# max-andr/joint-cnn-mrf

Measured on AMD Instinct MI355X. Metric: images/sec (720x480, K=9 joints) part-detector+spatial-model fwd, higher is better.
Workload: dtype f32(fp16x2 spectra, fft); 1 GPU; configs[1]: batch=64/GPU synthetic 480x720x3, part detector + spatial model forward + argmax, fp32; batch_per_gpu=64, global_batch=64, micro_batch=64, use_sm=True, collective=all_gather coords int32 [B,2,9]

## Files before the change

### joint-cnn-mrf_amd/csrc/conv_fft.hip

```cpp
#include <cmath>
#include <map>
#include <mutex>
#include <utility>
#include <vector>

#include "conv_fft_common.h"
#include "conv_fft_plan.h"

namespace jcm {
namespace cfft {

template <int KS, int NP>
__global__ __launch_bounds__(256) void weight_spectra_split_kernel(const float* __restrict__ w, uint4* __restrict__ Ws, int Cin, int Cout, int CoutP, int ntl, int NY, int NX,
                                                                   int round_bf16, float* __restrict__ wscale) {
  __shared__ cf twy[192][KS - 1], twx[KS];
  const int tid = threadIdx.x;
  const int kx = blockIdx.y;
#pragma unroll 1
  for (int k = tid; k < NY * (KS - 1) + KS; k += 256) {
    const bool isy = k < NY * (KS - 1);
    const int ky = k / (KS - 1), a = isy ? k % (KS - 1) + 1 : k - NY * (KS - 1);
    const int num = isy ? (ky * a) % NY : (kx * a) % NX, den = isy ? NY : NX;
    double sn, cs;
    sincospi(-2.0 * (double)num / (double)den, &sn, &cs);
    cf* dstw = isy ? &twy[ky][a - 1] : &twx[a];
    *dstw = cf{(float)cs, (float)sn};
  }
  __syncthreads();
  constexpr int CPT = 8;
  constexpr int NPP = NP == 5 ? 1 : 2;
  static_assert(NP == 2 || NP == 4 || NP == 5, "operand forms of the channel GEMM");
  float wmul = 1.f;
  if constexpr (NP >= 4) {
    int ex = 0;
    const float bound = wscale[0];
    if (bound > 0.f && bound < 3.0e38f) (void)frexpf(bound, &ex);
    wmul = ldexpf(1.f, 14 - ex);
    if (blockIdx.x == 0 && blockIdx.y == 0 && threadIdx.x == 0) wscale[1] = ldexpf(1.f, ex - 14);
  }
  const size_t e = (size_t)blockIdx.x * 256 + tid;
  if (e >= (size_t)(Cin / CPT) * CoutP) return;
  const int co = (int)(e % CoutP), cig = (int)(e / CoutP);
  cf ra[CPT][KS];
  const unsigned toff = (unsigned)(cig * CPT * Cout + (co < Cout ? co : Cout - 1));
#pragma unroll
  for (int c = 0; c < CPT; ++c)
#pragma unroll
    for (int a = 0; a < KS; ++a) ra[c][a] = cf{0.f, 0.f};
#pragma unroll 1
  for (int a = 0; a < KS; ++a) {
    cf sum[CPT];
#pragma unroll
    for (int c = 0; c < CPT; ++c) sum[c] = cf{0.f, 0.f};
#pragma unroll
    for (int b = 0; b < KS; ++b) {
      const float* tap = w + (size_t)((KS - 1 - a) * KS + (KS - 1 - b)) * Cin * Cout;
      const cf tw = twx[b];
#pragma unroll
      for (int c = 0; c < CPT; ++c) {
        float wv = tap[toff + (unsigned)(c * Cout)];
        wv = co < Cout ? wv : 0.f;
        if (round_bf16) wv = static_cast<float>(static_cast<__bf16>(wv));
        sum[c] = sfma(wv, tw, sum[c]);
      }
    }
#pragma unroll
    for (int c = 0; c < CPT; ++c)
#pragma unroll
      for (int aa = 0; aa < KS; ++aa) ra[c][aa] = aa == a ? sum[c] : ra[c][aa];
  }
  const int KC = Cin / 16, ntiles = CoutP / ntl;
  const int ci0 = cig * CPT, kc = ci0 >> 4, kg = (ci0 >> 3) & 1, nt = co / ntl, sn = co % ntl;
  const size_t fstride = NP == 5 ? (size_t)ntiles * (KC >> 1) * 8 * ntl : (size_t)ntiles * KC * (4 * NPP) * ntl;
  uint4* dst = Ws + (size_t)kx * NY * fstride +
               (NP == 5 ? ((size_t)nt * (KC >> 1) + (kc >> 1)) * 8 * ntl + ((size_t)(kc & 1) * 2 + kg) * ntl + sn :
                          ((size_t)nt * KC + kc) * (4 * NPP) * ntl + (size_t)kg * ntl + sn);
  typedef unsigned u32x4n __attribute__((ext_vector_type(4)));
  auto put = [](uint4* q, const uint4& v) __attribute__((always_inline)) { __builtin_nontemporal_store(u32x4n{v.x, v.y, v.z, v.w}, reinterpret_cast<u32x4n*>(q)); };
  auto emit = [&](uint4* d, const float (&xr)[CPT], const float (&xi)[CPT]) __attribute__((always_inline)) {
    if constexpr (NP == 5) {
      float x8[8];
#pragma unroll
      for (int c = 0; c < 8; ++c) x8[c] = xr[c % CPT];
      put(d, round8h(x8, wmul));
#pragma unroll
      for (int c = 0; c < 8; ++c) x8[c] = xi[c % CPT];
      put(d + (size_t)4 * ntl, round8h(x8, wmul));
    } else {
      uint4 u[NPP];
      float x8[8];
#pragma unroll
      for (int c = 0; c < 8; ++c) x8[c] = xr[c % CPT];
      if constexpr (NP == 4) split8h(x8, wmul, u);
      else split8<NPP>(x8, u);
#pragma unroll
      for (int p = 0; p < NPP; ++p) put(d + (size_t)p * 2 * ntl, u[p]);
#pragma unroll
      for (int c = 0; c < 8; ++c) x8[c] = xi[c % CPT];
      if constexpr (NP == 4) split8h(x8, wmul, u);
      else split8<NPP>(x8, u);
#pragma unroll
      for (int p = 0; p < NPP; ++p) put(d + (size_t)(NPP + p) * 2 * ntl, u[p]);
    }
  };
  for (int ky = 0; ky <= NY / 2; ++ky) {
    const int kp = ky == 0 ? 0 : NY - ky;
    float cs[KS - 1], sn_[KS - 1];
#pragma unroll
    for (int a = 1; a < KS; ++a) { const cf t = twy[ky][a - 1]; cs[a - 1] = t.x; sn_[a - 1] = -t.y; }
    float xr[CPT], xi[CPT], pr[CPT], pi_[CPT];
#pragma unroll
    for (int c = 0; c < CPT; ++c) {
      cf C = ra[c][0], S = cf{0.f, 0.f};
#pragma unroll
      for (int a = 1; a < KS; ++a) { C = sfma(cs[a - 1], ra[c][a], C); S = sfma(sn_[a - 1], ra[c][a], S); }
      xr[c] = C.x + S.y; xi[c] = C.y - S.x;
      pr[c] = C.x - S.y; pi_[c] = C.y + S.x;
    }
    emit(dst + (size_t)ky * fstride, xr, xi);
    if (kp != ky) emit(dst + (size_t)kp * fstride, pr, pi_);
  }
}

template <int TAPS>
__global__ __launch_bounds__(256) void weight_bound_kernel(const float* __restrict__ w, size_t pairs, int round_bf16, float* __restrict__ wmax) {
  __shared__ float red[4];
  float m = 0.f;
  for (size_t e = (size_t)blockIdx.x * 256 + threadIdx.x; e < pairs; e += (size_t)gridDim.x * 256) {
    float v[TAPS];
#pragma unroll
    for (int t = 0; t < TAPS; ++t) v[t] = w[(size_t)t * pairs + e];
    float sum = 0.f;
#pragma unroll
    for (int t = 0; t < TAPS; ++t) {
      float x = v[t];
      if (round_bf16) x = static_cast<float>(static_cast<__bf16>(x));
      sum += fabsf(x);
    }
    m = fmaxf(m, sum);
  }
  block_max_to<256>(m * 1.0001f, wmax, red, threadIdx.x);
}

struct Sizes { int NY, NX; };
static const int kLens[] = {20, 24, 28, 32, 36, 40, 50, 60, 64, 72, 96, 100, 128, 192};
static bool pick(int need, int* n) {
  for (int v : kLens)
    if (v >= need) { *n = v; return true; }
  return false;
}
static int tw_offset(int n) {
  int off = 0;
  for (int v : kLens) {
    if (v == n) return off;
    off += v;
  }
  return -1;
}
static bool sizes_of(int H, int W, int ks, Sizes* s, int circ = 0) {
  if (circ) {
    s->NY = H; s->NX = W;
    return (ks == 9 || ks == 5) && H > 8 && W > 8 && tw_offset(H) >= 0 && tw_offset(W) >= 0;
  }
  return (ks == 9 || ks == 5) && H + ks - 1 <= 192 && W + ks - 1 <= 192 && pick(H + 4, &s->NY) && pick(W + 4, &s->NX);
}
static int pad64(int c) { return (c + CB - 1) / CB * CB; }
static int padn(int c, int n) { return (c + n - 1) / n * n; }

int persistent_grid(const void* kernel, int ntiles, int threads, int dyn_lds) {
  static std::mutex mu;
  static std::map<std::pair<const void*, int>, int> cache;
  int dev = 0;
  (void)hipGetDevice(&dev);
  int resident = 0;
  {
    std::lock_guard<std::mutex> lk(mu);
    auto it = cache.find({kernel, dev});
    if (it != cache.end()) resident = it->second;
  }
  if (!resident) {
    int ncu = 256, per_cu = 0;
    (void)hipDeviceGetAttribute(&ncu, hipDeviceAttributeMultiprocessorCount, dev);
    if (hipOccupancyMaxActiveBlocksPerMultiprocessor(&per_cu, kernel, threads, (size_t)dyn_lds) != hipSuccess || per_cu < 1) per_cu = 1;
    resident = ncu * per_cu;
    std::lock_guard<std::mutex> lk(mu);
    cache[{kernel, dev}] = resident;
  }
  return resident < ntiles ? resident : ntiles;
}

static const cf* twiddle_table(int dev) {
  static std::mutex mu;
  static std::map<int, cf*> tabs;
  std::lock_guard<std::mutex> lk(mu);
  auto it = tabs.find(dev);
  if (it != tabs.end()) return it->second;
  std::vector<float> h;
  for (int n : kLens)
    for (int k = 0; k < n; ++k) {
      const double ang = 2.0 * 3.14159265358979323846 * (double)k / (double)n;
      h.push_back((float)std::cos(ang));
      h.push_back((float)std::sin(ang));
    }
  cf* d = nullptr;
  if (hipMalloc(reinterpret_cast<void**>(&d), h.size() * sizeof(float)) != hipSuccess) return nullptr;
  if (hipMemcpy(d, h.data(), h.size() * sizeof(float), hipMemcpyHostToDevice) != hipSuccess) { (void)hipFree(d); return nullptr; }
  tabs[dev] = d;
  return d;
}

}

using namespace cfft;

bool conv_fft_supported(const ConvArgs& a, int ks, int circ) {
  Sizes s;
  return a.Cin % CB == 0 && a.Cin >= CB && a.Cout >= 1 && a.B >= 1 && sizes_of(a.H, a.W, ks, &s, circ);
}
static bool operand_form(int np) { return np == kFftBf16x2 || np == kFftFp16x2 || np == kFftFp16x1; }
size_t conv_fft_weight_bytes(int H, int W, int ks, int Cin, int Cout, int np, int circ) {
  Sizes s;
  if (!sizes_of(H, W, ks, &s, circ)) return 0;
  return cgemm_split_w_bytes(np, s.NY * (s.NX / 2 + 1), Cin, Cout);
}
hipError_t conv_fft_pack_weights(const float* w_hwio, void* wf, int H, int W, int ks, int Cin, int Cout, int np, bool round_bf16, hipStream_t st, float* wscale, int circ,
                                 const float* bound_from) {
  Sizes s;
  if (!sizes_of(H, W, ks, &s, circ) || Cin % 16 || !operand_form(np) || (np >= 4 && !wscale) || (np == kFftFp16x1 && Cin % 32)) return hipErrorInvalidValue;
  const int ntl = cgemm_split_ntile(np, Cout), CoutP = padn(Cout, ntl);
  const size_t cpt = 8;
  const dim3 grid((unsigned)(((size_t)Cin / cpt * CoutP + 255) / 256), (unsigned)(s.NX / 2 + 1));
  uint4* dst = static_cast<uint4*>(wf);
  const int rb = round_bf16 ? 1 : 0;
  if (np >= 4 && bound_from) {
    if (hipError_t e = hipMemcpyAsync(wscale, bound_from, sizeof(float), hipMemcpyDeviceToDevice, st); e != hipSuccess) return e;
  } else if (np >= 4) {
    if (hipError_t e = hipMemsetAsync(wscale, 0, 2 * sizeof(float), st); e != hipSuccess) return e;
    const size_t pairs = (size_t)Cin * Cout;
    const dim3 bgrid((unsigned)((pairs + 255) / 256 > 1024 ? 1024 : (pairs + 255) / 256));
    if (ks == 9) hipLaunchKernelGGL(weight_bound_kernel<81>, bgrid, dim3(256), 0, st, w_hwio, pairs, rb, wscale);
    else hipLaunchKernelGGL(weight_bound_kernel<25>, bgrid, dim3(256), 0, st, w_hwio, pairs, rb, wscale);
  }
#define WS_LAUNCH(KS, NPV) hipLaunchKernelGGL((weight_spectra_split_kernel<KS, NPV>), grid, dim3(256), 0, st, w_hwio, dst, Cin, Cout, CoutP, ntl, s.NY, s.NX, rb, wscale)
  if (ks == 9) {
    if (np == 2) WS_LAUNCH(9, 2); else if (np == 4) WS_LAUNCH(9, 4); else WS_LAUNCH(9, 5);
  } else {
    if (np == 2) WS_LAUNCH(5, 2); else if (np == 4) WS_LAUNCH(5, 4); else WS_LAUNCH(5, 5);
  }
#undef WS_LAUNCH
  return hipGetLastError();
}
bool conv_fft_fusable(const ConvArgs& a, int ks, int ks_next) {
  Sizes s, n;
  return sizes_of(a.H, a.W, ks, &s) && sizes_of(a.H, a.W, ks_next, &n) && s.NX == n.NX && a.Cout % CB == 0;
}
static size_t align256(size_t v) { return (v + 255) & ~size_t(255); }
FftHandover16 conv_fft_handover16(int B, int NXH, int H, int C) {
  FftHandover16 h;
  h.words_off = align256((size_t)B * NXH * H * C * 4);
  h.bytes = h.words_off + (size_t)B * H * (C / CB) * sizeof(float);
  return h;
}
size_t conv_fft_handover_bytes(const ConvArgs& a, int ks, bool h16) {
  Sizes s;
  if (!sizes_of(a.H, a.W, ks, &s)) return 0;
  const int NXH = s.NX / 2 + 1;
  const size_t f32 = (size_t)a.B * NXH * a.H * a.Cout * sizeof(cf);
  const size_t b16 = h16 ? conv_fft_handover16(a.B, NXH, a.H, a.Cout).bytes : 0;
  return f32 > b16 ? f32 : b16;
}
bool conv_fft_win_gather_supported(int win, int Cin, bool fft_reg) { return fft_reg && cfft_rows_fwd_win_reg_supported(win, Cin); }
bool conv_fft_win_scatter_supported(int win, int Cout, bool fft_reg) { return fft_reg && win == 32 && Cout % 64 == 0; }
bool conv_fft_pool_fusable(const ConvArgs& a, int ks, int ks_next) {
  Sizes s, n;
  return sizes_of(a.H, a.W, ks, &s) && sizes_of((a.H + 1) / 2, (a.W + 1) / 2, ks_next, &n) && cfft_rows_inv_pool_fwd_supported(s.NX, n.NX, a.Cout);
}
size_t conv_fft_pool_handover_bytes(const ConvArgs& a, int ks_next) {
  Sizes n;
  if (!sizes_of((a.H + 1) / 2, (a.W + 1) / 2, ks_next, &n)) return 0;
  return (size_t)a.B * (n.NX / 2 + 1) * ((a.H + 1) / 2) * a.Cout * sizeof(cf);
}
bool conv_fft_merge_fusable(const ConvArgs& a, int ks, int ks_next, const FftMerge& m, bool fft_reg, bool h16) {
  Sizes s;
  if (!conv_fft_fusable(a, ks, ks_next) || !sizes_of(a.H, a.W, ks, &s)) return false;
  const bool reg = fft_reg && cfft_rows_inv_merge_fwd_reg_supported(s.NX, a, m, (ks - 1) / 2);
  return h16 ? reg : (reg || cfft_rows_inv_merge_fwd_supported(s.NX, a, m));
}
bool conv_fft_geometry(int H, int W, int ks, int B, int Cout, int np, int* NY, int* NX, int* MT, int circ) {
  Sizes s;
  if (!sizes_of(H, W, ks, &s, circ)) return false;
  *NY = s.NY; *NX = s.NX; *MT = cgemm_split_mtile(np, B, Cout);
  return true;
}
size_t conv_fft_logits_weight_bytes(int H, int W, int Cin) {
  Sizes s;
  return sizes_of(H, W, 9, &s) ? cfft_logits_rows_operand_bytes(s.NX, Cin) : 0;
}
hipError_t conv_fft_logits_pack(const float* w_hwio, void* aop, int H, int W, int Cin, int Cout, hipStream_t st, float* wscale) {
  Sizes s;
  if (!sizes_of(H, W, 9, &s) || Cin % 16 || Cout > 16 || !wscale) return hipErrorInvalidValue;
  if (hipError_t e = hipMemsetAsync(wscale, 0, 2 * sizeof(float), st); e != hipSuccess) return e;
  const size_t pairs = (size_t)Cin * Cout;
  const dim3 bgrid((unsigned)((pairs + 255) / 256 > 1024 ? 1024 : (pairs + 255) / 256));
  hipLaunchKernelGGL(weight_bound_kernel<81>, bgrid, dim3(256), 0, st, w_hwio, pairs, 0, wscale);
  if (!cfft_logits_rows_pack(s.NX, w_hwio, aop, Cin, Cout, wscale, st)) return hipErrorInvalidValue;
  return hipGetLastError();
}

static void carve(FftPlan* p, size_t t, size_t xs, size_t yf, size_t sc_fwd, size_t sc_inv) {
  FftRegion* const regions[] = {&p->T, &p->Xs, &p->Yf, &p->t16_fwd, &p->t16_inv};
  const size_t bytes[] = {t, xs, yf, sc_fwd, sc_inv};
  size_t off = 0;
  for (int i = 0; i < 5; ++i) {
    regions[i]->off = off;
    regions[i]->bytes = bytes[i];
    off += align256(bytes[i]);
  }
  p->total = off;
}
FftPlan conv_fft_plan(const FftArgs& a, int ks, int np, int pool_ks_next) {
  FftPlan p;
  Sizes s, n;
  p.ok = a.tiles ? sizes_of(a.H / 2, a.W / 2, ks, &s) : sizes_of(a.H, a.W, ks, &s, a.circ);
  if (!p.ok) return p;
  p.ks = ks; p.np = np;
  p.NY = s.NY; p.NX = s.NX; p.NXH = s.NX / 2 + 1; p.F = s.NY * p.NXH;
  if (pool_ks_next && sizes_of((a.H + 1) / 2, (a.W + 1) / 2, pool_ks_next, &n)) p.NX_next = n.NX;
  p.opad = (ks - 1) / 2 + (a.circ ? 4 : 0);
  p.norm = 1.0f / (float)(s.NY * s.NX);
  p.map = a;
  p.map.CoutP = pad64(a.Cout);
  p.col = p.map;
  if (a.tiles) { p.col.B = 4 * a.B; p.col.H = s.NY; p.col.W = a.W / 2; p.col.tiles = 0; }
  p.inv = p.col;
  if (a.tiles) p.inv.H = a.H / 2;
  if (a.circ) { p.inv.H = a.H - 8; p.inv.W = a.W - 8; }
  const FftArgs& c = p.col;
  p.ldy = padn(c.Cout, cgemm_split_ntile(np, c.Cout));
  if (p.ldy < pad64(c.Cout)) p.ldy = pad64(c.Cout);
  p.MT = cgemm_split_mtile(np, c.B, c.Cout);
  p.inv_cb = s.NY > 100 ? 32 : 64;
  const size_t cop = pad64(c.Cout), cmax = (size_t)c.Cin > cop ? c.Cin : cop;
  const size_t bp = (size_t)(c.B + p.MT - 1) / p.MT * p.MT;
  carve(&p, (size_t)c.B * p.NXH * c.H * cmax * sizeof(cf), (size_t)p.F * bp * c.Cin * 4 * cgemm_split_parts(np), (size_t)p.F * c.B * p.ldy * sizeof(cf),
        (size_t)c.B * c.H * (c.Cin / CB) * sizeof(float), (size_t)c.B * p.NXH * (cop / p.inv_cb) * sizeof(float));
  return p;
}
FftPlan conv_fft_logits_plan(const FftArgs& a) {
  FftPlan p;
  Sizes s;
  p.ok = sizes_of(a.H, a.W, 9, &s);
  if (!p.ok) return p;
  p.ks = 9; p.np = kFftFp16x2;
  p.NY = s.NY; p.NX = s.NX; p.NXH = s.NX / 2 + 1; p.F = s.NY * p.NXH;
  p.opad = 4;
  p.norm = 1.0f / (float)s.NX;
  p.map = a;
  p.map.CoutP = pad64(a.Cout);
  p.col = p.inv = p.map;
  carve(&p, (size_t)a.B * a.H * p.NXH * CB * sizeof(cf), 0, 0, 0, 0);
  return p;
}
hipError_t conv_fft_plan_twiddles(FftPlan* p) {
  int dev = 0;
  if (hipError_t e = hipGetDevice(&dev); e != hipSuccess) return e;
  const cf* twb = twiddle_table(dev);
  if (!twb) return hipErrorOutOfMemory;
  p->twx = twb + tw_offset(p->NX);
  p->twy = twb + tw_offset(p->NY);
  p->twx_next = p->NX_next ? twb + tw_offset(p->NX_next) : nullptr;
  return hipSuccess;
}
size_t conv_fft_workspace_bytes(const FftArgs& a, int ks, int np) {
  const FftPlan p = conv_fft_plan(a, ks, np);
  return p.ok ? p.total : 0;
}
size_t conv_fft_xs_bytes(const FftArgs& a0, int ks, int np) {
  FftArgs a = a0;
  a.tiles = 0;
  const FftPlan p = conv_fft_plan(a, ks, np);
  return p.ok ? align256(p.Xs.bytes) : 0;
}

const char* conv_fft_refusal(const FftPlan& p, FftLayout in, FftLayout out, const FftLink& k, int t16) {
  const FftArgs& a = p.map;
  if (!p.ok) return "no transform size for this map and kernel size";
  if (a.Cin % CB || a.Cin < CB || a.Cout < 1 || a.B < 1) return "input channels in whole blocks of 64, at least one output channel and one image";
  if (out == kFftBf16Planar && a.Cout % 8) return "planar bf16 output needs whole units of 8 channels";
  if (!operand_form(p.np)) return "operand forms of the channel GEMM: 2, 4, 5";
  if (p.np == kFftFp16x1 && a.Cin % 32) return "the one-part operand stages 32 input channels at a time";
  if (a.circ && (k.t_in || k.t_next || k.merge || in != kFftF32Nhwc || out != kFftF32Nhwc)) return "windows take fp32 NHWC on both sides and no hand-over";
  if ((k.next.pool || k.next.merge) && (!k.t_next || (k.next.pool && k.next.merge))) return "a pool or merge hand-over needs t_next, and only one of the two";
  const bool h16 = t16 && ((k.t_next && k.next.merge && !k.t_in) || (k.t_in && !k.t_next));
  if ((k.t_in || k.t_next) && !h16 && (in != kFftF32Nhwc || out != kFftF32Nhwc)) return "a 32-bit hand-over takes fp32 NHWC tensors on both sides";
  if (k.t_next && a.Cout % CB) return "a hand-over needs output channels in whole blocks of 64";
  if (t16 && p.np != kFftFp16x1) return "16-bit T needs the one-part operand form";
  if (t16 && (in == kFftF32Nhwc || out == kFftF32Nhwc)) return "16-bit T needs bf16 tensors on both sides";
  if (t16 && (k.xs || ((k.t_in || k.t_next) && !h16))) return "16-bit T keeps no spectra and hands over only across the merge";
  if (k.merge && in == kFftBf16Planar) return "the merge reads NHWC";
  if (k.xs_ready && !k.xs) return "ready spectra without their buffer";
  if (k.t_next && k.next.pool && !p.NX_next) return "no transform size for the pooled map";
  return nullptr;
}
const char* conv_fft_tiles_refusal(const FftPlan& p, FftLayout in, FftLayout, const FftLink& k) {
  const FftArgs& a = p.map;
  if (!a.tiles) return "not planned as tiles";
  if (p.np != kFftFp16x2 || in != kFftF32Nhwc) return "tiles exist on fp32 handles (operand form 4, fp32 NHWC input)";
  if (k.t_in || k.merge || k.xs || k.xs_ready || k.win_map) return "tiles read their own map: no hand-over in, no merge, no kept spectra, no windows";
  if (!k.t_next || !k.next.pool || k.next.merge) return "tiles feed the pool hand-over and nothing else";
  if (!a.fft_reg) return "tiles exist as register kernels only";
  if (p.ks != 5 || k.next.ks_next != 5) return "tiles exist for a 5x5 layer in front of a 5x5 layer";
  if (a.circ || a.win_map || a.B < 1) return "tiles of whole maps, at least one image";
  if (!conv_fft_pool_fusable(a, p.ks, k.next.ks_next)) return "no pool hand-over for this pair of layers";
  if (a.H % 4 || a.W % 4 || !p.ok || !cfft_tiles_supported(p.NY, p.NX, a)) return "tiles exist for the model's 120 x 180 map geometry";
  return nullptr;
}
const char* conv_fft_logits_refusal(const FftPlan& p, int ks, int np, FftLayout in, FftLayout out, const FftLink& k, int common) {
  const FftArgs& a = p.map;
  if (ks != 9 || np != kFftFp16x2 || in != kFftF32Nhwc || out != kFftF32Nhwc) return "logits rows: a 9x9 layer of an fp32 handle, fp32 NHWC on both sides";
  if (a.circ || a.tiles || a.win_map || k.win_map || k.win_scatter) return "logits rows: whole maps, no windows, no tiles";
  if (!p.ok || !conv_fft_supported(a, 9) || !cfft_logits_rows_supported(p.NX, a)) return "logits rows: 96-point rows, at most 64 rows and 16 output channels";
  if (!k.t_in || k.t_in_16) return "logits rows read a 32-bit row-transformed input";
  if (k.t_next || k.next.pool || k.next.merge || k.merge || k.xs || k.xs_ready) return "logits rows hand nothing over and keep no spectra";
  if (common) return "logits rows scale each image by its own word";
  return nullptr;
}

namespace {
struct Run {
  const FftPlan& p;
  cf* T;
  void* Xs;
  cf* Yf;
  Fp16Scale sc;
  float yshift, yinv;
  hipStream_t st;
  bool reg() const { return p.map.fft_reg != 0; }
};
Fp16Scale device_scale(const FftPlan& p, const FftScale* in, float hf, void* work) {
  Fp16Scale sc;
  if (p.np < 4 || !in) return sc;
  sc.tmax = in->tmax; sc.tmax_next = in->tmax_next; sc.winv = in->winv; sc.common = in->common; sc.t16 = in->t16;
  sc.hf = hf;
  sc.nb = p.col.B;
  if (sc.t16) {
    sc.t16_fwd = p.at<float>(work, p.t16_fwd);
    sc.t16_inv = p.at<float>(work, p.t16_inv);
    sc.t16_cb = p.inv_cb;
  }
  return sc;
}
hipError_t refuse(const char** why, const char* reason) {
  if (why) *why = reason;
  return hipErrorInvalidValue;
}
hipError_t not_launched(const char** why, const char* reason) {
  const hipError_t e = hipGetLastError();
  return e != hipSuccess ? e : refuse(why, reason);
}

bool pass_rows_fwd(const Run& r, FftLayout in, const FftMerge* merge) {
  const FftPlan& p = r.p;
  const FftArgs& a = p.map;
  if (a.tiles) return cfft_rows_fwd_tile_reg(p.NY, p.NX, a, r.T, r.sc.tmax, r.st);
  if (merge) return (r.reg() && cfft_rows_fwd_merge_reg(p.NX, a, *merge, in, r.T, r.sc.tmax, r.st, r.sc.t16_fwd)) || cfft_rows_fwd_merge(p.NX, a, *merge, in, r.T, p.twx, r.sc.tmax, r.st, r.sc.t16_fwd);
  if (a.win_map) return cfft_rows_fwd_win_reg(p.NX, a, r.T, r.sc.tmax, r.st);
  return (r.reg() && cfft_rows_fwd_reg(p.NX, a, in, r.T, r.sc.tmax, r.st, r.sc.t16_fwd)) || cfft_rows_fwd(p.NX, a, in, r.T, p.twx, r.sc.tmax, r.st, r.sc.t16_fwd);
}
bool pass_cols_fwd(const Run& r, const cf* Tin) { return cfft_cols_fwd(r.p.NY, r.p.col, r.p.np, Tin, r.Xs, r.p.twy, r.p.NXH, r.p.MT, r.sc, r.st); }
hipError_t pass_gemm(const Run& r, hipEvent_t g0, hipEvent_t g1) {
  const FftArgs& c = r.p.col;
  if (g0 && hipEventRecord(g0, r.st) != hipSuccess) return hipErrorUnknown;
  if (hipError_t e = cgemm_split(r.Xs, c.wp, r.Yf, r.p.np, r.p.F, c.B, c.Cin, c.Cout, r.p.ldy, r.st, r.yshift); e != hipSuccess) return e;
  if (g1 && hipEventRecord(g1, r.st) != hipSuccess) return hipErrorUnknown;
  return hipSuccess;
}
bool pass_cols_inv(const Run& r) {
  const FftPlan& p = r.p;
  if (r.reg() && p.inv_cb == 64 && cfft_cols_inv_reg(p.NY, p.inv, r.Yf, r.T, p.NXH, p.ldy, p.opad, r.st, r.sc.t16_inv, r.yinv)) return true;
  if (p.map.tiles) return false;
  return cfft_cols_inv(p.NY, p.inv, r.Yf, r.T, p.twy, p.NXH, p.ldy, p.opad, r.st, r.sc.t16_inv, r.yinv);
}
bool pass_rows_inv(const Run& r, FftLayout out, const FftLink& k, bool lds_only = false) {
  const FftPlan& p = r.p;
  const FftArgs& a = p.map;
  cf* Tn = static_cast<cf*>(k.t_next);
  if (lds_only) return cfft_rows_inv(p.NX, p.inv, out, r.T, p.twx, p.opad, p.norm, r.sc, r.st);
  if (a.tiles) return cfft_rows_inv_pool_tile_reg(p.NY, p.NX, a, r.T, Tn, p.norm, r.sc, r.st);
  if (Tn && k.next.pool) return cfft_rows_inv_pool_fwd(p.NX, p.NX_next, a, r.T, Tn, p.twx, p.twx_next, p.opad, p.norm, r.sc, r.st);
  if (Tn && k.next.merge) {
    if (r.sc.t16) return r.reg() && cfft_rows_inv_merge_fwd_reg(p.NX, a, *k.next.merge, r.T, Tn, p.opad, p.norm, r.sc, r.st, conv_fft_handover16(a.B, p.NXH, a.H, a.Cout).words(Tn));
    return (r.reg() && cfft_rows_inv_merge_fwd_reg(p.NX, a, *k.next.merge, r.T, Tn, p.opad, p.norm, r.sc, r.st)) || cfft_rows_inv_merge_fwd(p.NX, a, *k.next.merge, r.T, Tn, p.twx, p.opad, p.norm, r.sc, r.st);
  }
  if (Tn) return (r.reg() && cfft_rows_inv_fwd_reg(p.NX, a, r.T, Tn, p.opad, p.norm, r.sc, r.st)) || cfft_rows_inv_fwd(p.NX, a, r.T, Tn, p.twx, p.opad, p.norm, r.sc, r.st);
  if ((p.inv.rows_mfma & 1) && cfft_rows_inv_mfma(p.NX, p.inv, out, r.T, p.opad, p.norm, r.sc, r.st)) return true;
  if (r.reg() && cfft_rows_inv_reg(p.NX, p.inv, out, r.T, p.opad, p.norm, r.sc, r.st)) return true;
  if (p.inv.win_scatter) return false;
  return cfft_rows_inv(p.NX, p.inv, out, r.T, p.twx, p.opad, p.norm, r.sc, r.st);
}
const char* scale_refusal(const FftPlan& p, const FftScale* sc, const FftLink& k) {
  if (p.np < 4) return nullptr;
  if (!sc || !sc->tmax || !sc->winv) return "scaled operand forms need the scale words of the input and of the filter spectra";
  if (k.t_next && !sc->tmax_next) return "a hand-over needs the scale words of the next layer";
  return nullptr;
}
}

hipError_t conv_fft_f32(FftPlan p, FftLayout in, FftLayout out, void* work, const FftLink& k, hipEvent_t g0, hipEvent_t g1, hipStream_t st, const FftScale* scp, const char** why) {
  const int t16 = p.np >= 4 && scp ? scp->t16 : 0;
  if (const char* no = p.map.tiles ? conv_fft_tiles_refusal(p, in, out, k) : conv_fft_refusal(p, in, out, k, t16)) return refuse(why, no);
  if (const char* no = scale_refusal(p, scp, k)) return refuse(why, no);
  if (hipError_t e = conv_fft_plan_twiddles(&p); e != hipSuccess) return e;
  Run r{p, p.at<cf>(work, p.T), k.xs ? k.xs : p.at<void>(work, p.Xs), p.at<cf>(work, p.Yf), device_scale(p, scp, (float)p.col.H, work), 0.f, 0.f, st};
  if (r.sc.t16 && k.t_in) r.sc.t16_fwd = conv_fft_handover16(p.col.B, p.NXH, p.col.H, p.col.Cin).words(k.t_in);
  r.yshift = r.sc.t16 ? cgemm_split_y16_shift(p.col.Cin) : 0.f;
  r.yinv = r.yshift != 0.f ? 1.0f / r.yshift : 0.f;
  if (!k.xs_ready) {
    if (!k.t_in && !pass_rows_fwd(r, in, k.merge)) return not_launched(why, "no forward row kernel for this case");
    if (!pass_cols_fwd(r, k.t_in ? static_cast<const cf*>(k.t_in) : r.T)) return not_launched(why, "no forward column kernel for this operand form and scale");
  }
  if (hipError_t e = hipGetLastError(); e != hipSuccess) return e;
  if (hipError_t e = pass_gemm(r, g0, g1); e != hipSuccess) return e;
  if (!pass_cols_inv(r)) return not_launched(why, "no inverse column kernel for this case");
  if (!pass_rows_inv(r, out, k)) return not_launched(why, p.inv.win_scatter ? "the scatter into the map exists in the register kernel only" : "no kernel for this hand-over");
  return hipGetLastError();
}

hipError_t conv_fft_logits_f32(FftPlan p, int ks, int np, FftLayout in, FftLayout out, void* work, const FftLink& k, hipEvent_t g0, hipEvent_t g1, hipStream_t st,
                               const FftScale* scp, const char** why) {
  if (const char* no = conv_fft_logits_refusal(p, ks, np, in, out, k, scp ? scp->common : 0)) return refuse(why, no);
  if (const char* no = scale_refusal(p, scp, k)) return refuse(why, no);
  if (hipError_t e = conv_fft_plan_twiddles(&p); e != hipSuccess) return e;
  const Run r{p, p.at<cf>(work, p.T), nullptr, nullptr, device_scale(p, scp, 1.f, work), 0.f, 0.f, st};
  if (g0 && hipEventRecord(g0, st) != hipSuccess) return hipErrorUnknown;
  if (!cfft_logits_rows(p.NX, p.map, static_cast<const cf*>(k.t_in), p.map.wp, r.sc.tmax, r.T, st)) return not_launched(why, "no logits-rows kernel for this case");
  if (hipError_t e = hipGetLastError(); e != hipSuccess) return e;
  if (g1 && hipEventRecord(g1, st) != hipSuccess) return hipErrorUnknown;
  if (!pass_rows_inv(r, out, k, true)) return not_launched(why, "no inverse row kernel for this case");
  return hipGetLastError();
}

hipError_t conv_fft_spectra(const FftArgs& a0, int ks, int np, void* work, void* xs, hipStream_t st, float* tmax, int common, const char** why) {
  FftArgs a = a0;
  a.tiles = 0;
  FftPlan p = conv_fft_plan(a, ks, np);
  if (!p.ok || !conv_fft_supported(a, ks, a.circ)) return refuse(why, "no transform size for this map and kernel size, or channels not in whole blocks of 64");
  if (!xs || (np >= 4 && !tmax)) return refuse(why, "spectra need their buffer and, in the scaled operand forms, the scale word");
  if (hipError_t e = conv_fft_plan_twiddles(&p); e != hipSuccess) return e;
  FftScale in;
  in.tmax = tmax; in.common = common;
  const Run r{p, p.at<cf>(work, p.T), xs, nullptr, device_scale(p, &in, (float)a.H, work), 0.f, 0.f, st};
  if (!pass_rows_fwd(r, kFftF32Nhwc, nullptr)) return not_launched(why, "no forward row kernel for this case");
  if (!pass_cols_fwd(r, r.T)) return not_launched(why, "no forward column kernel for this operand form and scale");
  return hipGetLastError();
}

}
```

### joint-cnn-mrf_amd/csrc/conv_fft_cols.hip

```cpp
#include "conv_fft_common.h"

namespace jcm {
namespace cfft {

template <int NY, int NP, bool T16 = false>
__global__ __launch_bounds__(colfwd_threads<NY>()) void cols_fwd_split_kernel(const cf* __restrict__ T, uint4* __restrict__ Xs, const cf* __restrict__ twg, int B, int H, int KC, int MT,
                                                            int mtiles, const float* __restrict__ tmax, int common, const float* __restrict__ t16, int ntiles) {
  constexpr int IMG = colimg<NY>(), CH = IMG * 16, NTC = colfwd_threads<NY>(), NPP = NP == 5 ? 1 : 2;
  constexpr int CPV = T16 ? 4 : 2;
  constexpr int NV = NY * CH / CPV, KV = (NV + NTC - 1) / NTC, VPR = CH / CPV, VPI = 16 / CPV;
  extern __shared__ __attribute__((aligned(16))) char smem_cf[];
  cf* buf = reinterpret_cast<cf*>(smem_cf);
  cf* tw = buf + NY * CH;
  float4* buf4 = reinterpret_cast<float4*>(buf);
  const int tid = threadIdx.x;
  const int NG = (B + IMG - 1) / IMG;
  twiddles<NY, NTC>(tw, twg, tid);
  __shared__ float xsc[IMG];
  uint4 pre[KV];
  float psc[KV];
  auto coords = [&](int tile, int& kc, int& kx, int& b0, int& nimg) __attribute__((always_inline)) {
    const int g = tile % NG, kk = tile / NG;
    kc = kk % KC; kx = kk / KC;
    b0 = g * IMG; nimg = min(IMG, B - b0);
  };
  auto prefetch = [&](int tile) __attribute__((always_inline)) {
    int kc, kx, b0, nimg;
    coords(tile, kc, kx, b0, nimg);
    const uint4* src = reinterpret_cast<const uint4*>(T) + (((size_t)kx * KC + kc) * B + b0) * H * VPI;
#pragma unroll
    for (int i = 0; i < KV; ++i) {
      const int t = tid + i * NTC, y = t / VPR, v = t % VPR, img = v / VPI, cv = v % VPI;
      const bool ok = t < NV && y < H && img < nimg;
      pre[i] = ok ? src[((size_t)img * H + y) * VPI + cv] : make_uint4(0u, 0u, 0u, 0u);
      if constexpr (T16) psc[i] = ok ? t16[((size_t)(b0 + img) * (KC >> 2) + (kc >> 2)) * H + y] : 0.f;
    }
  };
  int tile = blockIdx.x;
  if (tile < ntiles) prefetch(tile);
  for (; tile < ntiles; tile += gridDim.x) {
    int kc, kx, b0, nimg;
    coords(tile, kc, kx, b0, nimg);
#pragma unroll
    for (int i = 0; i < KV; ++i) {
      const int t = tid + i * NTC;
      if (t < NV) {
        if constexpr (T16) {
          const cf a = unpack_h2(pre[i].x, psc[i]), b2 = unpack_h2(pre[i].y, psc[i]), c2 = unpack_h2(pre[i].z, psc[i]), d2 = unpack_h2(pre[i].w, psc[i]);
          buf4[2 * t] = make_float4(a.x, a.y, b2.x, b2.y);
          buf4[2 * t + 1] = make_float4(c2.x, c2.y, d2.x, d2.y);
        } else {
          buf4[t] = make_float4(__uint_as_float(pre[i].x), __uint_as_float(pre[i].y), __uint_as_float(pre[i].z), __uint_as_float(pre[i].w));
        }
      }
    }
    if constexpr (NP >= 4)
      if (tid < IMG) xsc[tid] = tid < nimg ? fp16_scale(tmax_of(tmax, b0 + tid, B, common), (float)H) : 1.f;
    __syncthreads();
    if (tile + (int)gridDim.x < ntiles) prefetch(tile + (int)gridDim.x);
    fft<NY, -1, CH, NTC>(buf, tw, tid);
    const int mt = b0 / MT, r0 = b0 - mt * MT;
    for (int it = tid; it < NY * 2 * IMG; it += NTC) {
      const int img = it % IMG, kg = (it / IMG) & 1, ky = it / (2 * IMG);
      const cf* z = buf + pos<NY>(ky) * CH + img * 16 + kg * 8;
      float re[8], im[8];
#pragma unroll
      for (int e = 0; e < 8; ++e) { re[e] = z[e].x; im[e] = z[e].y; }
      uint4 ur[NPP], ui[NPP];
      if constexpr (NP == 5) {
        const float xscale = xsc[img];
        ur[0] = round8h(re, xscale);
        ui[0] = round8h(im, xscale);
      } else if constexpr (NP == 4) {
        const float xscale = xsc[img];
        split8h(re, xscale, ur);
        split8h(im, xscale, ui);
      } else {
        split8<NPP>(re, ur);
        split8<NPP>(im, ui);
      }
      const size_t f = (size_t)kx * NY + ky;
      if constexpr (NP == 5) {
        uint4* dst = Xs + (((f * mtiles + mt) * (KC >> 1) + (kc >> 1)) * 8 + (size_t)(kc & 1) * 2 + kg) * MT + r0 + img;
        st_stream(dst, ur[0]);
        st_stream(dst + (size_t)4 * MT, ui[0]);
      } else {
        uint4* dst = Xs + (((f * mtiles + mt) * KC + kc) * (4 * NPP) + kg) * MT + r0 + img;
#pragma unroll
        for (int p = 0; p < NPP; ++p) {
          st_stream(dst + (size_t)(0 * NPP + p) * 2 * MT, ur[p]);
          st_stream(dst + (size_t)(1 * NPP + p) * 2 * MT, ui[p]);
        }
      }
    }
    __syncthreads();
  }
}

template <int NY, bool T16 = false>
__global__ __launch_bounds__(colinv_threads<NY>()) void cols_inv_kernel(const cf* __restrict__ Yf, cf* __restrict__ T, const cf* __restrict__ twg, int B, int H, int NXH, int C, int ldy,
                                                      int pad, float* __restrict__ t16, float yinv) {
  constexpr int CH = colblk<NY>(), CB = CH, NTC = colinv_threads<NY>();
  __shared__ cf buf[NY * CH];
  __shared__ cf tw[NY];
  const int tid = threadIdx.x;
  const int cblk = blockIdx.x % (C / CB), bk = blockIdx.x / (C / CB);
  const int kx = bk % NXH, b = bk / NXH;
  twiddles<NY, NTC>(tw, twg, tid);
  for (int t = tid; t < NY * CH; t += NTC) {
    const int ky = t / CH, v = t % CH;
    const size_t src = ((size_t)(kx * NY + ky) * B + b) * ldy + cblk * CB + v;
    if constexpr (T16) buf[t] = unpack_h2(reinterpret_cast<const unsigned*>(Yf)[src], 1.f);
    else buf[t] = Yf[src];
  }
  __syncthreads();
  fft<NY, 1, CH, NTC>(buf, tw, tid);
  if constexpr (T16) {
    constexpr int KM = (NY * CH + NTC - 1) / NTC;
    __shared__ float red[NTC / 64];
    cf val[KM];
    float m = 0.f;
#pragma unroll
    for (int i = 0; i < KM; ++i) {
      const int t = tid + i * NTC, y = t / CH, v = t % CH;
      val[i] = cf{0.f, 0.f};
      if (t < H * CH) {
        val[i] = buf[pos<NY>(y + pad) * CH + v];
        m = fmaxf(m, fmaxf(fabsf(val[i].x), fabsf(val[i].y)));
      }
    }
    const float s = bfp_scale(block_max_all<NTC>(m, red, tid));
    unsigned* dst = reinterpret_cast<unsigned*>(T);
#pragma unroll
    for (int i = 0; i < KM; ++i) {
      const int t = tid + i * NTC, y = t / CH, v = t % CH;
      if (t < H * CH) st_stream(&dst[((size_t)(b * H + y) * NXH + kx) * C + cblk * CB + v], pack_h2(val[i].x * s, val[i].y * s));
    }
    if (tid == 0) t16[((size_t)b * (C / CB) + cblk) * NXH + kx] = (1.0f / s) * yinv;
  } else {
    for (int t = tid; t < H * CH; t += NTC) {
      const int y = t / CH, v = t % CH;
      st_stream(&T[((size_t)(b * H + y) * NXH + kx) * C + cblk * CB + v], buf[pos<NY>(y + pad) * CH + v]);
    }
  }
}


template <int NY> static bool launch_cols_fwd(const FftArgs& a, int np, const cf* T, void* Xs, const cf* tw, int NXH, int MT, const Fp16Scale& sc, hipStream_t st) {
  constexpr int IMG = colimg<NY>();
  constexpr int lds = (NY * IMG * 16 + NY) * (int)sizeof(cf);
  const int KC = a.Cin / 16, mtiles = (a.B + MT - 1) / MT;
  const int ntiles = NXH * KC * ((a.B + IMG - 1) / IMG);
  static LdsAttr attr2, attr4, attr5, attr5h;
  const dim3 blk(colfwd_threads<NY>());
#define COLS_FWD(KERNEL, ATTR, ...)                                                                              \
  do {                                                                                                           \
    if (ATTR.ensure(reinterpret_cast<const void*>(KERNEL), lds) != hipSuccess) return false;                      \
    const dim3 grid((unsigned)persistent_grid(reinterpret_cast<const void*>(KERNEL), ntiles, (int)blk.x, lds));  \
    hipLaunchKernelGGL(KERNEL, grid, blk, lds, st, T, static_cast<uint4*>(Xs), tw, a.B, a.H, KC, MT, mtiles, __VA_ARGS__, ntiles); \
  } while (0)
  if (np == 5 && sc.t16_fwd) {
    if (!sc.tmax || (KC & 3)) return false;
    COLS_FWD((cols_fwd_split_kernel<NY, 5, true>), attr5h, sc.tmax, sc.common, sc.t16_fwd);
  } else if (np == 5) {
    if (!sc.tmax || (KC & 1)) return false;
    COLS_FWD((cols_fwd_split_kernel<NY, 5>), attr5, sc.tmax, sc.common, (const float*)nullptr);
  } else if (np == 2) {
    COLS_FWD((cols_fwd_split_kernel<NY, 2>), attr2, (const float*)nullptr, 0, (const float*)nullptr);
  } else if (np == 4) {
    if (!sc.tmax) return false;
    COLS_FWD((cols_fwd_split_kernel<NY, 4>), attr4, sc.tmax, sc.common, (const float*)nullptr);
  } else {
    return false;
  }
#undef COLS_FWD
  return true;
}
template <int NY> static void launch_cols_inv(const FftArgs& a, const cf* Yf, cf* T, const cf* tw, int NXH, int ldy, int pad, hipStream_t st, float* t16, float y16_inv) {
  const dim3 grid(a.B * NXH * (a.CoutP / colblk<NY>())), blk(colinv_threads<NY>());
  if (t16) hipLaunchKernelGGL((cols_inv_kernel<NY, true>), grid, blk, 0, st, Yf, T, tw, a.B, a.H, NXH, a.CoutP, ldy, pad, t16, y16_inv);
  else hipLaunchKernelGGL((cols_inv_kernel<NY, false>), grid, blk, 0, st, Yf, T, tw, a.B, a.H, NXH, a.CoutP, ldy, pad, nullptr, 0.f);
}
bool cfft_cols_fwd(int NY, const FftArgs& a, int np, const cf* T, void* Xs, const cf* tw, int NXH, int MT, const Fp16Scale& sc, hipStream_t st) {
  bool e = false;
#define CALL(N) e = launch_cols_fwd<N>(a, np, T, Xs, tw, NXH, MT, sc, st)
  CFFT_BY_SIZE(NY, CALL)
#undef CALL
  return e;
}
bool cfft_cols_inv(int NY, const FftArgs& a, const cf* Yf, cf* T, const cf* tw, int NXH, int ldy, int pad, hipStream_t st, float* t16, float y16_inv) {
#define CALL(N) launch_cols_inv<N>(a, Yf, T, tw, NXH, ldy, pad, st, t16, y16_inv)
  CFFT_BY_SIZE(NY, CALL)
#undef CALL
  return true;
}

}
}
```

### joint-cnn-mrf_amd/csrc/conv_fft_common.h

```cpp
#pragma once
#include "fft_lds.h"
#include "kernels.h"

namespace jcm {
namespace cfft {
using namespace fftl;
constexpr int CB = 64, NT = 256;
constexpr int kParMax = 512;

template <int N> struct Plan;
template <> struct Plan<192> { static constexpr int R1 = 8, R2 = 8, R3 = 3; };
template <> struct Plan<128> { static constexpr int R1 = 8, R2 = 4, R3 = 4; };
template <> struct Plan<100> { static constexpr int R1 = 4, R2 = 5, R3 = 5; };
template <> struct Plan<96> { static constexpr int R1 = 8, R2 = 12, R3 = 1; };
template <> struct Plan<72> { static constexpr int R1 = 8, R2 = 3, R3 = 3; };
template <> struct Plan<64> { static constexpr int R1 = 8, R2 = 8, R3 = 1; };
template <> struct Plan<60> { static constexpr int R1 = 4, R2 = 15, R3 = 1; };
template <> struct Plan<50> { static constexpr int R1 = 5, R2 = 10, R3 = 1; };
template <> struct Plan<40> { static constexpr int R1 = 8, R2 = 5, R3 = 1; };
template <> struct Plan<36> { static constexpr int R1 = 4, R2 = 3, R3 = 3; };
template <> struct Plan<32> { static constexpr int R1 = 8, R2 = 4, R3 = 1; };
template <> struct Plan<28> { static constexpr int R1 = 4, R2 = 7, R3 = 1; };
template <> struct Plan<24> { static constexpr int R1 = 8, R2 = 3, R3 = 1; };
template <> struct Plan<20> { static constexpr int R1 = 4, R2 = 5, R3 = 1; };
template <int N> __device__ __forceinline__ int pos(int n) {
  using P = Plan<N>;
  if constexpr (P::R3 == 1) return (n % P::R1) * (N / P::R1) + n / P::R1;
  else return (n % P::R1) * (N / P::R1) + ((n / P::R1) % P::R2) * (N / (P::R1 * P::R2)) + n / (P::R1 * P::R2);
}

template <int N, int R, int L, int S, int CH, int NTH = NT>
__device__ __forceinline__ void stage(cf* buf, const cf* tw, int tid) {
  constexpr int M = L / R, BF = N / R;
  for (int t = tid; t < BF * CH; t += NTH) {
    const int bf = t / CH, v = t % CH;
    const int blk = bf / M, k = bf - blk * M;
    cf* p = buf + (blk * L + k) * CH + v;
    cf x[R];
#pragma unroll
    for (int m = 0; m < R; ++m) x[m] = p[m * M * CH];
    Dft<R, S>::run(x);
    if (M > 1) {
#pragma unroll
      for (int m = 1; m < R; ++m) {
        cf w = tw[(N / L) * k * m];
        if (S < 0) w.y = -w.y;
        x[m] = cmul(x[m], w);
      }
    }
#pragma unroll
    for (int m = 0; m < R; ++m) p[m * M * CH] = x[m];
  }
}
template <int N, int S, int CH, int NTH = NT>
__device__ __forceinline__ void fft(cf* buf, const cf* tw, int tid) {
  using P = Plan<N>;
  stage<N, P::R1, N, S, CH, NTH>(buf, tw, tid);
  __syncthreads();
  stage<N, P::R2, N / P::R1, S, CH, NTH>(buf, tw, tid);
  __syncthreads();
  if constexpr (P::R3 > 1) {
    stage<N, P::R3, N / (P::R1 * P::R2), S, CH, NTH>(buf, tw, tid);
    __syncthreads();
  }
}
template <int N, int NTH = NT>
__device__ __forceinline__ void twiddles(cf* tw, const cf* __restrict__ twg, int tid) {
  for (int k = tid; k < N; k += NTH) tw[k] = twg[k];
}


__device__ __forceinline__ float bfp_scale(float m) {
  int e = 0;
  if (!(m > 1.0e-30f && m < 3.0e38f)) return 1.f;
  (void)frexpf(m, &e);
  return ldexpf(1.f, 15 - e);
}
__device__ __forceinline__ unsigned pack_h2(float a, float b) {
  return (unsigned)__builtin_bit_cast(unsigned short, static_cast<_Float16>(a)) | ((unsigned)__builtin_bit_cast(unsigned short, static_cast<_Float16>(b)) << 16);
}
__device__ __forceinline__ cf unpack_h2(unsigned u, float s) {
  return cf{static_cast<float>(__builtin_bit_cast(_Float16, (unsigned short)(u & 0xffffu))) * s, static_cast<float>(__builtin_bit_cast(_Float16, (unsigned short)(u >> 16))) * s};
}
__device__ __forceinline__ cf unpack_h2_mix_s(unsigned u, float s) {
  cf r;
  asm("v_fma_mix_f32 %0, %1, %2, 0 op_sel_hi:[1,0,0]" : "=v"(r.x) : "v"(u), "s"(s));
  asm("v_fma_mix_f32 %0, %1, %2, 0 op_sel:[1,0,0] op_sel_hi:[1,0,0]" : "=v"(r.y) : "v"(u), "s"(s));
  return r;
}
__device__ __forceinline__ cf unpack_h2_mix_v(unsigned u, float s) {
  cf r;
  asm("v_fma_mix_f32 %0, %1, %2, 0 op_sel_hi:[1,0,0]" : "=v"(r.x) : "v"(u), "v"(s));
  asm("v_fma_mix_f32 %0, %1, %2, 0 op_sel:[1,0,0] op_sel_hi:[1,0,0]" : "=v"(r.y) : "v"(u), "v"(s));
  return r;
}
__device__ __forceinline__ float wave_max(float m) {
#pragma unroll
  for (int o = 32; o > 0; o >>= 1) m = fmaxf(m, __shfl_xor(m, o));
  return m;
}
template <int NTH>
__device__ __forceinline__ float block_max_all(float m, float* red, int tid) {
  m = wave_max(m);
  if ((tid & 63) == 0) red[tid >> 6] = m;
  __syncthreads();
  float r = red[0];
#pragma unroll
  for (int w = 1; w < NTH / 64; ++w) r = fmaxf(r, red[w]);
  return r;
}
__device__ __forceinline__ cf bf16pair(unsigned bits) { return cf{__uint_as_float(bits << 16), __uint_as_float(bits & 0xffff0000u)}; }
__device__ __forceinline__ size_t t_fwd_index(int k, int cblk, int v, int b, int y, int B, int H, int C) {
  return ((((size_t)k * (C >> 4) + cblk * 4 + (v >> 3)) * B + b) * H + y) * 8 + (v & 7);
}
template <int NX, int NTH = NT>
__device__ __forceinline__ float rows_fwd_store(const cf* buf, cf* __restrict__ T, int tid, int cblk, int b, int y, int B, int H, int C) {
  constexpr int CH = CB / 2, NXH = NX / 2 + 1;
  float4* dst = reinterpret_cast<float4*>(T);
  float m = 0.f;
  for (int t = tid; t < NXH * CH; t += NTH) {
    const int k = t / CH, v = t % CH;
    const cf zk = buf[pos<NX>(k) * CH + v], zn = buf[pos<NX>(k == 0 ? 0 : NX - k) * CH + v];
    const float4 o = make_float4(0.5f * (zk.x + zn.x), 0.5f * (zk.y - zn.y), 0.5f * (zk.y + zn.y), -0.5f * (zk.x - zn.x));
    dst[t_fwd_index(k, cblk, v, b, y, B, H, C)] = o;
    m = fmaxf(fmaxf(m, fmaxf(fabsf(o.x), fabsf(o.y))), fmaxf(fabsf(o.z), fabsf(o.w)));
  }
  return m;
}

template <int NX, int NTH = NT>
__device__ __forceinline__ float rows_fwd_store16(const cf* buf, void* T, float* __restrict__ tinv, float* red2, int tid, int cblk, int b, int y, int B, int H, int C) {
  constexpr int CH = CB / 2, NXH = NX / 2 + 1, K = (NXH * CH + NTH - 1) / NTH;
  uint2* dst = reinterpret_cast<uint2*>(T);
  float4 o[K];
  float m = 0.f;
#pragma unroll
  for (int i = 0; i < K; ++i) {
    const int t = tid + i * NTH, k = t / CH, v = t % CH;
    o[i] = make_float4(0.f, 0.f, 0.f, 0.f);
    if (t < NXH * CH) {
      const cf zk = buf[pos<NX>(k) * CH + v], zn = buf[pos<NX>(k == 0 ? 0 : NX - k) * CH + v];
      o[i] = make_float4(0.5f * (zk.x + zn.x), 0.5f * (zk.y - zn.y), 0.5f * (zk.y + zn.y), -0.5f * (zk.x - zn.x));
      m = fmaxf(fmaxf(m, fmaxf(fabsf(o[i].x), fabsf(o[i].y))), fmaxf(fabsf(o[i].z), fabsf(o[i].w)));
    }
  }
  const float s = bfp_scale(block_max_all<NTH>(m, red2, tid));
#pragma unroll
  for (int i = 0; i < K; ++i) {
    const int t = tid + i * NTH, k = t / CH, v = t % CH;
    if (t < NXH * CH) dst[t_fwd_index(k, cblk, v, b, y, B, H, C)] = make_uint2(pack_h2(o[i].x * s, o[i].y * s), pack_h2(o[i].z * s, o[i].w * s));
  }
  if (tid == 0) tinv[((size_t)b * (C / CB) + cblk) * H + y] = 1.0f / s;
  return m;
}

constexpr int kFp16TargetExp = 15;
static_assert(kFp16TargetExp <= 15, "sqrt(2) * 2^kFp16TargetExp must stay below fp16's largest number 65504");
__device__ __forceinline__ int fp16_exp(float tmax, float hf) {
  const float bound = tmax * hf;
  int e = 0;
  if (bound > 0.f && bound < 3.0e38f) (void)frexpf(bound, &e);
  return e;
}
__device__ __forceinline__ int fp16_k(float tmax, float hf) { const int k = kFp16TargetExp - fp16_exp(tmax, hf); return k > 126 ? 126 : (k < -126 ? -126 : k); }
__device__ __forceinline__ float fp16_scale(float tmax, float hf) { return ldexpf(1.f, fp16_k(tmax, hf)); }
__device__ __forceinline__ float fp16_unscale(float tmax, float hf) { return ldexpf(1.f, -fp16_k(tmax, hf)); }
__device__ __forceinline__ float tmax_of(const float* __restrict__ tmax, int b, int nb, int common) {
  if (!common) return tmax[b];
  float m = 0.f;
  for (int i = 0; i < nb; ++i) m = fmaxf(m, tmax[i]);
  return m;
}
__device__ __forceinline__ void wave_max_stash(float m, float* red) {
  m = wave_max(m);
  if ((threadIdx.x & 63) == 0) red[threadIdx.x >> 6] = m;
}
template <int NTH>
__device__ __forceinline__ void stash_to_word(const float* red, float* dst) {
  if (threadIdx.x == 0) {
    float m = red[0];
#pragma unroll
    for (int w = 1; w < NTH / 64; ++w) m = fmaxf(m, red[w]);
    if (m > 0.f) atomicMax(reinterpret_cast<unsigned*>(dst), __float_as_uint(m));
  }
}
template <int NTH>
__device__ __forceinline__ void block_max_to(float m, float* dst, float* red, int tid) {
  m = wave_max(m);
  if ((tid & 63) == 0) red[tid >> 6] = m;
  __syncthreads();
  if (tid == 0) {
    for (int w = 1; w < NTH / 64; ++w) m = fmaxf(m, red[w]);
    if (m > 0.f) atomicMax(reinterpret_cast<unsigned*>(dst), __float_as_uint(m));
  }
}
template <int NX> constexpr int rows_threads() { return NX >= 128 ? 512 : NX >= 72 ? 384 : 256; }
template <int NY> constexpr int colblk() { return NY > 100 ? 32 : 64; }
template <int NY> constexpr int colimg() { return NY > 96 ? 4 : 8; }
template <int NY> constexpr int colfwd_threads() { return NY * colimg<NY>() * 16 >= 8192 ? 1024 : NY * colimg<NY>() * 16 >= 4096 ? 512 : 256; }
template <int NY> constexpr int colinv_threads() { return NY * colblk<NY>() >= 4096 ? 512 : 256; }
__device__ __forceinline__ void split8h(const float (&x)[8], float scale, uint4 (&out)[2]) {
  unsigned short h[2][8];
#pragma unroll
  for (int e = 0; e < 8; ++e) {
    float v = x[e] * scale;
#pragma unroll
    for (int p = 0; p < 2; ++p) {
      const _Float16 q = static_cast<_Float16>(v);
      h[p][e] = __builtin_bit_cast(unsigned short, q);
      v = v - static_cast<float>(q);
    }
  }
#pragma unroll
  for (int p = 0; p < 2; ++p)
    out[p] = make_uint4((unsigned)h[p][0] | ((unsigned)h[p][1] << 16), (unsigned)h[p][2] | ((unsigned)h[p][3] << 16), (unsigned)h[p][4] | ((unsigned)h[p][5] << 16),
                        (unsigned)h[p][6] | ((unsigned)h[p][7] << 16));
}
__device__ __forceinline__ uint4 round8h(const float (&x)[8], float scale) {
  unsigned short h[8];
#pragma unroll
  for (int e = 0; e < 8; ++e) h[e] = __builtin_bit_cast(unsigned short, static_cast<_Float16>(x[e] * scale));
  return make_uint4((unsigned)h[0] | ((unsigned)h[1] << 16), (unsigned)h[2] | ((unsigned)h[3] << 16), (unsigned)h[4] | ((unsigned)h[5] << 16), (unsigned)h[6] | ((unsigned)h[7] << 16));
}
template <int NP>
__device__ __forceinline__ void split8(const float (&x)[8], uint4 (&out)[NP]) {
  unsigned short h[NP][8];
#pragma unroll
  for (int e = 0; e < 8; ++e) {
    float v = x[e];
#pragma unroll
    for (int p = 0; p < NP; ++p) {
      const __bf16 q = static_cast<__bf16>(v);
      h[p][e] = __builtin_bit_cast(unsigned short, q);
      v = v - static_cast<float>(q);
    }
  }
#pragma unroll
  for (int p = 0; p < NP; ++p)
    out[p] = make_uint4((unsigned)h[p][0] | ((unsigned)h[p][1] << 16), (unsigned)h[p][2] | ((unsigned)h[p][3] << 16), (unsigned)h[p][4] | ((unsigned)h[p][5] << 16),
                        (unsigned)h[p][6] | ((unsigned)h[p][7] << 16));
}
#define CFFT_BY_SIZE(N, CALL)                    \
  switch (N) {                                   \
    case 20: CALL(20); break;                    \
    case 24: CALL(24); break;                    \
    case 28: CALL(28); break;                    \
    case 32: CALL(32); break;                    \
    case 36: CALL(36); break;                    \
    case 40: CALL(40); break;                    \
    case 50: CALL(50); break;                    \
    case 60: CALL(60); break;                    \
    case 64: CALL(64); break;                    \
    case 72: CALL(72); break;                    \
    case 96: CALL(96); break;                    \
    case 100: CALL(100); break;                  \
    case 128: CALL(128); break;                  \
    default: CALL(192); break;                   \
  }

int persistent_grid(const void* kernel, int ntiles, int threads, int dyn_lds = 0);

bool cfft_rows_fwd(int NX, const FftArgs& a, FftLayout layout, cf* T, const cf* tw, float* tmax, hipStream_t st, float* t16 = nullptr);
bool cfft_rows_fwd_merge(int NX, const FftArgs& a, const FftMerge& m, FftLayout in_layout, cf* T, const cf* tw, float* tmax, hipStream_t st, float* t16 = nullptr);
bool cfft_cols_fwd(int NY, const FftArgs& a, int np, const cf* T, void* Xs, const cf* tw, int NXH, int MT, const Fp16Scale& sc, hipStream_t st);
bool cfft_cols_inv(int NY, const FftArgs& a, const cf* Yf, cf* T, const cf* tw, int NXH, int ldy, int pad, hipStream_t st, float* t16 = nullptr, float y16_inv = 0.f);
bool cfft_rows_inv(int NX, const FftArgs& a, FftLayout layout, const cf* T, const cf* tw, int pad, float norm, const Fp16Scale& sc, hipStream_t st);
bool cfft_rows_inv_fwd(int NX, const FftArgs& a, const cf* T, cf* Tn, const cf* tw, int pad, float norm, const Fp16Scale& sc, hipStream_t st);
bool cfft_rows_inv_reg(int NX, const FftArgs& a, FftLayout layout, const cf* T, int pad, float norm, const Fp16Scale& sc, hipStream_t st);
bool cfft_rows_inv_fwd_reg(int NX, const FftArgs& a, const cf* T, cf* Tn, int pad, float norm, const Fp16Scale& sc, hipStream_t st);
bool cfft_rows_fwd_reg(int NX, const FftArgs& a, FftLayout layout, cf* T, float* tmax, hipStream_t st, float* t16);
bool cfft_rows_fwd_win_reg(int NX, const FftArgs& a, cf* T, float* tmax, hipStream_t st);
bool cfft_rows_fwd_win_reg_supported(int NX, int Cin);
bool cfft_tiles_supported(int NY, int NX, const FftArgs& a);
bool cfft_rows_fwd_tile_reg(int NY, int NX, const FftArgs& a, cf* T, float* tmax, hipStream_t st);
bool cfft_rows_inv_pool_tile_reg(int NY, int NX, const FftArgs& a, const cf* T, cf* Tn, float norm, const Fp16Scale& sc, hipStream_t st);
bool cfft_rows_fwd_merge_reg(int NX, const FftArgs& a, const FftMerge& m, FftLayout in_layout, cf* T, float* tmax, hipStream_t st, float* t16);
bool cfft_cols_inv_reg(int NY, const FftArgs& a, const cf* Yf, cf* T, int NXH, int ldy, int pad, hipStream_t st, float* t16, float y16_inv = 0.f);
bool cfft_rows_inv_pool_fwd(int NXI, int NXO, const FftArgs& a, const cf* T, cf* Tn, const cf* twi, const cf* two, int pad, float norm, const Fp16Scale& sc, hipStream_t st);
bool cfft_rows_inv_merge_fwd(int NX, const FftArgs& a, const FftMerge& m, const cf* T, cf* Tn, const cf* tw, int pad, float norm, const Fp16Scale& sc, hipStream_t st);
bool cfft_rows_inv_merge_fwd_reg(int NX, const FftArgs& a, const FftMerge& m, const cf* T, cf* Tn, int pad, float norm, const Fp16Scale& sc, hipStream_t st, float* t16n = nullptr);
bool cfft_rows_inv_merge_fwd_reg_supported(int NX, const ConvArgs& a, const FftMerge& m, int pad);
bool cfft_rows_inv_pool_fwd_supported(int NXI, int NXO, int Cout);
bool cfft_rows_inv_mfma(int NX, const FftArgs& a, FftLayout layout, const cf* T, int pad, float norm, const Fp16Scale& sc, hipStream_t st);
bool cfft_rows_inv_merge_fwd_supported(int NX, const ConvArgs& a, const FftMerge& m);
bool cfft_logits_rows_supported(int NX, const FftArgs& a);
size_t cfft_logits_rows_operand_bytes(int NX, int Cin);
bool cfft_logits_rows_pack(int NX, const float* w_hwio, void* aop, int Cin, int Cout, float* wscale, hipStream_t st);
bool cfft_logits_rows(int NX, const FftArgs& a, const cf* T, const void* aop, const float* tmax, cf* S, hipStream_t st);
}
}
```

### joint-cnn-mrf_amd/csrc/conv_fft_plan.h

```cpp
#pragma once
#include "kernels.h"

namespace jcm {

typedef float fft_cf __attribute__((ext_vector_type(2)));

struct FftRegion {
  size_t off = 0, bytes = 0;
};
struct FftPlan {
  bool ok = false;
  int ks = 0, np = 0;
  int NY = 0, NX = 0, NXH = 0, F = 0;
  int NX_next = 0;
  int opad = 0;
  int MT = 0, ldy = 0, inv_cb = 64;
  float norm = 0.f;
  FftArgs map;
  FftArgs col;
  FftArgs inv;
  FftRegion T, Xs, Yf, t16_fwd, t16_inv;
  size_t total = 0;
  const fft_cf *twx = nullptr, *twy = nullptr, *twx_next = nullptr;

  template <class X> X* at(void* work, const FftRegion& r) const { return reinterpret_cast<X*>(static_cast<char*>(work) + r.off); }
};
FftPlan conv_fft_plan(const FftArgs& a, int ks, int np, int pool_ks_next = 0);
FftPlan conv_fft_logits_plan(const FftArgs& a);
hipError_t conv_fft_plan_twiddles(FftPlan* p);

struct FftHandover16 {
  size_t words_off = 0, bytes = 0;
  float* words(const void* t) const { return reinterpret_cast<float*>(static_cast<char*>(const_cast<void*>(t)) + words_off); }
};
FftHandover16 conv_fft_handover16(int B, int NXH, int H, int C);

const char* conv_fft_refusal(const FftPlan& p, FftLayout in, FftLayout out, const FftLink& link, int t16);
const char* conv_fft_tiles_refusal(const FftPlan& p, FftLayout in, FftLayout out, const FftLink& link);
const char* conv_fft_logits_refusal(const FftPlan& p, int ks, int np, FftLayout in, FftLayout out, const FftLink& link, int common);

hipError_t conv_fft_f32(FftPlan p, FftLayout in, FftLayout out, void* work, const FftLink& link, hipEvent_t g0, hipEvent_t g1, hipStream_t st, const FftScale* sc,
                        const char** why);
hipError_t conv_fft_logits_f32(FftPlan p, int ks, int np, FftLayout in, FftLayout out, void* work, const FftLink& link, hipEvent_t g0, hipEvent_t g1, hipStream_t st,
                               const FftScale* sc, const char** why);

}
```

### joint-cnn-mrf_amd/csrc/conv_fft_reg_inv.hip

```cpp
#include "fft_reg_rows.h"

namespace jcm {
namespace cfft {

template <int NX, int LAYOUT, bool T16>
__global__ __launch_bounds__(256) __attribute__((amdgpu_waves_per_eu(NX >= 64 ? 2 : 4, NX >= 64 ? 2 : 8))) void rows_inv_reg_kernel(const void* __restrict__ T, void* __restrict__ out, const float* __restrict__ bias,
                                                                                              const float* __restrict__ scale, const float* __restrict__ shift, int relu_bn,
                                                                                              int nrows, int H, int W, int C, int Cout, int pad, float norm0, Fp16Scale sc,
                                                                                              int smH, int smW, int sTY, int sTX) {
  constexpr int M = NX / 2;
  __shared__ __attribute__((aligned(16))) unsigned stage[LAYOUT != 0 ? 4 * M * 64 : 4];
  int h, p;
  size_t by;
  pair_coords<true>(C >> 1, h, p, by);
  if (by >= (size_t)nrows) return;
  const int b = (int)(by / H), c = 2 * p;
  const bool odd = h != 0;
  const float sg = odd ? -1.f : 1.f;
  cf u[M];
  if constexpr (T16) {
    TInvRow16<NX> load;
    load.scales(sc, b, c, C);
    load.request(T, by, C, p);
    inv_rows_load2<NX, 0>(u, sg, odd, load);
  } else {
    inv_rows_load2<NX, 0>(u, sg, odd, TInvRow32<NX>(T, by, C, p));
  }
  const Epilogue<false, true> act(bias, scale, shift, relu_bn, c, Cout, scale_undo(norm0, sc, b, scale_common(sc)));
  const bool two = c + 1 < Cout;
  step1<M, 1>(u);
  const int lane = threadIdx.x & 63;
  int sc_row = -1, sc_x0 = 0;
  if (LAYOUT == 0 && sTX > 0) {
    const int bw = (int)(by / H), yv = (int)(by % H);
    const int tx = bw % sTX, ty = (bw / sTX) % sTY, bi = bw / (sTX * sTY), ym = ty * H + yv;
    sc_row = ym < smH ? bi * smH + ym : -1;
    sc_x0 = tx * W;
  }
  unsigned* wst = stage + (LAYOUT != 0 ? (threadIdx.x >> 6) * (M * 64) : 0);
  auto store = [&](int m, int xo, cf z) __attribute__((always_inline)) {
    const cf v = act(z);
    if constexpr (LAYOUT == 0) {
      if (sTX > 0) {
        const int xm = sc_x0 + xo;
        if (sc_row >= 0 && xm < smW) st_stream(reinterpret_cast<cf*>(static_cast<float*>(out) + ((size_t)sc_row * smW + xm) * Cout + c), v);
      } else {
        st_stream(reinterpret_cast<cf*>(static_cast<float*>(out) + (by * W + xo) * Cout + c), v);
      }
    } else {
      typedef __bf16 bf16x2 __attribute__((ext_vector_type(2)));
      wst[(m * 2 + h) * 32 + (lane >> 1)] = __builtin_bit_cast(unsigned, bf16x2{static_cast<__bf16>(v.x), static_cast<__bf16>(v.y)});
    }
  };
  if (two || LAYOUT != 0) inv_rows_out2<NX, 0, LAYOUT != 0>(u, h, W, pad, store);
  if constexpr (LAYOUT != 0) {
    __builtin_amdgcn_fence(__ATOMIC_RELEASE, "wavefront");
    __builtin_amdgcn_wave_barrier();
    const int y = (int)(by % H);
    const int c0 = c - (lane >> 1) * 2;
    const uint4* rd = reinterpret_cast<const uint4*>(wst);
#pragma unroll 4
    for (int q = lane; q < M * 16; q += 64) {
      const int m = q >> 4, hh = (q >> 3) & 1, j = q & 7;
      const int xo = 2 * m + hh - pad, cu = c0 + 8 * j;
      if (xo >= 0 && xo < W && cu < Cout) {
        __bf16* o = LAYOUT == 1 ? static_cast<__bf16*>(out) + (by * W + xo) * Cout + cu
                                : static_cast<__bf16*>(out) + (((size_t)b * (Cout >> 3) + (cu >> 3)) * H * W + (size_t)y * W + xo) * 8;
        *reinterpret_cast<uint4*>(o) = rd[q];
      }
    }
  }
}

template <int NY, bool T16>
__global__ __launch_bounds__(256) __attribute__((amdgpu_waves_per_eu(NY >= 64 ? 2 : 3, NY >= 64 ? 2 : 8))) void cols_inv_reg_kernel(const cf* __restrict__ Yf, void* __restrict__ T, int B, int H, int NXH, int C, int ldy,
                                                                                              int pad, float* __restrict__ t16, float yinv) {
  static_assert(NY % 2 == 0, "ky pairs");
  constexpr int R1 = RPlan<NY>::R1, R2 = RPlan<NY>::R2;
  const size_t g = (size_t)blockIdx.x * 256 + threadIdx.x;
  const int c = (int)(g % C);
  const unsigned bk = (unsigned)__builtin_amdgcn_readfirstlane((int)(g / C));
  const int kx = (int)(bk % (unsigned)NXH), b = (int)(bk / (unsigned)NXH);
  if (b >= B) return;
  const bool odd = (c & 1) != 0;
  cf x[NY];
  if constexpr (T16) {
    const uint2* src = reinterpret_cast<const uint2*>(reinterpret_cast<const unsigned*>(Yf) + ((size_t)kx * NY * B + b) * ldy + (c & ~1));
    const size_t kstep = (size_t)B * ldy / 2;
    uint2 raw[NY / 2];
#pragma unroll
    for (int i = 0; i < NY / 2; ++i) raw[i] = src[(size_t)(2 * i + (odd ? 1 : 0)) * kstep];
    __builtin_amdgcn_sched_barrier(0);
#pragma unroll
    for (int i = 0; i < NY / 2; ++i) {
      const unsigned keep = odd ? raw[i].y : raw[i].x, recv = lane_pair_swap(odd ? raw[i].x : raw[i].y);
      x[2 * i] = unpack_h2(odd ? recv : keep, 1.f);
      x[2 * i + 1] = unpack_h2(odd ? keep : recv, 1.f);
    }
  } else {
    const cf* src = Yf + ((size_t)kx * NY * B + b) * ldy + c;
#pragma unroll
    for (int ky = 0; ky < NY; ++ky) x[ky] = src[(size_t)ky * B * ldy];
  }
  step1<NY, 1>(x);
  step2_inplace<NY, 1, 0>(x);
  if constexpr (T16) {
    float m = 0.f;
#pragma unroll
    for (int i = 0; i < NY; ++i) {
      const int y = (i / R2) + R1 * (i % R2) - pad;
      if (y >= 0 && y < H) m = fmaxf(m, fmaxf(fabsf(x[i].x), fabsf(x[i].y)));
    }
    const float s = bfp_scale(wave_max(m));
    if ((threadIdx.x & 63) == 0) t16[((size_t)b * (C >> 6) + (c >> 6)) * NXH + kx] = (1.0f / s) * yinv;
    uint2* dst = reinterpret_cast<uint2*>(reinterpret_cast<unsigned*>(T) + ((size_t)b * H * NXH + kx) * C + (c & ~1));
    const size_t ystep = (size_t)NXH * C / 2;
#pragma unroll
    for (int k = 0; k < NY; k += 2) {
      const int ia = R2 * (k % R1) + k / R1, ib = R2 * ((k + 1) % R1) + (k + 1) / R1;
      const unsigned va = pack_h2(x[ia].x * s, x[ia].y * s), vb = pack_h2(x[ib].x * s, x[ib].y * s);
      const unsigned recv = lane_pair_swap(odd ? va : vb);
      const int y = k - pad + (odd ? 1 : 0);
      if (y >= 0 && y < H) st_stream(dst + (size_t)y * ystep, make_uint2(odd ? recv : va, odd ? vb : recv));
    }
  } else {
#pragma unroll
    for (int i = 0; i < NY; ++i) {
      const int y = (i / R2) + R1 * (i % R2) - pad;
      if (y >= 0 && y < H) st_stream(reinterpret_cast<cf*>(T) + ((size_t)(b * H + y) * NXH + kx) * C + c, x[i]);
    }
  }
}
bool cfft_cols_inv_reg(int NY, const FftArgs& a, const cf* Yf, cf* T, int NXH, int ldy, int pad, hipStream_t st, float* t16, float y16_inv) {
  if (a.CoutP % 64 || ((y16_inv != 0.f) != (t16 != nullptr)) || (t16 && ldy % 2)) return false;
  const size_t threads = (size_t)a.B * NXH * a.CoutP;
  const dim3 grid((unsigned)((threads + 255) / 256)), blk(256);
#define CI_LAUNCH(N)                                                                                                                                             \
  do {                                                                                                                                                           \
    if (t16) hipLaunchKernelGGL((cols_inv_reg_kernel<N, true>), grid, blk, 0, st, Yf, static_cast<void*>(T), a.B, a.H, NXH, a.CoutP, ldy, pad, t16, y16_inv);            \
    else hipLaunchKernelGGL((cols_inv_reg_kernel<N, false>), grid, blk, 0, st, Yf, static_cast<void*>(T), a.B, a.H, NXH, a.CoutP, ldy, pad, nullptr, 0.f);          \
  } while (0)
  switch (NY) {
    case 64: CI_LAUNCH(64); break;
    case 36: CI_LAUNCH(36); break;
    case 32: CI_LAUNCH(32); break;
    case 20: CI_LAUNCH(20); break;
    default: return false;
  }
#undef CI_LAUNCH
  return true;
}

template <int NX> static bool launch_rows_inv_reg(const FftArgs& a, FftLayout layout, const cf* T, int pad, float norm, const Fp16Scale& sc, hipStream_t st) {
  const int nrows = a.B * a.H;
  if (a.win_scatter && (layout != kFftF32Nhwc || sc.t16_inv)) return false;
  if ((a.Cout & 1) || a.CoutP % 64) return false;
  const size_t threads = (size_t)nrows * a.CoutP;
  const dim3 grid((unsigned)((threads + 255) / 256)), blk(256);
  const bool h16 = sc.t16_inv != nullptr;
  const WinGeom wout = a.win_scatter ? a.win : WinGeom{};
#define RR_LAUNCH(L, H16) hipLaunchKernelGGL((rows_inv_reg_kernel<NX, L, H16>), grid, blk, 0, st, T, a.out, a.bias, a.scale, a.shift, a.relu_bn, nrows, a.H, a.W, a.CoutP, a.Cout, pad, norm, sc, wout.H, wout.W, wout.TY, wout.TX)
  if (layout == kFftF32Nhwc && !h16) RR_LAUNCH(0, false);
  else if (layout == kFftBf16Nhwc && h16 && a.Cout % 8 == 0) RR_LAUNCH(1, true);
  else if (layout == kFftBf16Nhwc && a.Cout % 8 == 0) RR_LAUNCH(1, false);
  else if (layout == kFftBf16Planar && h16 && a.Cout % 8 == 0) RR_LAUNCH(2, true);
  else if (layout == kFftBf16Planar && a.Cout % 8 == 0) RR_LAUNCH(2, false);
  else return false;
#undef RR_LAUNCH
  return true;
}
bool cfft_rows_inv_reg(int NX, const FftArgs& a, FftLayout layout, const cf* T, int pad, float norm, const Fp16Scale& sc, hipStream_t st) {
  if (NX == 96) return launch_rows_inv_reg<96>(a, layout, T, pad, norm, sc, st);
  if (NX == 32 && layout == kFftF32Nhwc) return launch_rows_inv_reg<32>(a, layout, T, pad, norm, sc, st);
  if (NX == 50) return launch_rows_inv_reg<50>(a, layout, T, pad, norm, sc, st);
  if (NX == 28) return launch_rows_inv_reg<28>(a, layout, T, pad, norm, sc, st);
  return false;
}

}
}
```

### joint-cnn-mrf_amd/csrc/conv_route.hip

```cpp
#include <string>

#include "conv_fft_plan.h"
#include "ctx.h"

namespace jcm {

bool takes_strip(const ConvLayer* L, int B, int H, int W) {
  if (!L->wp_bf16 || L->thin_bf16 || conv_igemm_bf16_bn(L->cout, L->ks) != 256) return false;
  ConvArgs a = conv_args(L, B, H, W);
  a.CoutP = L->coutp_bf16;
  a.out_planar = 1;
  return conv_strip_bf16_supported(a, L->ks);
}

bool takes_c5strip(const ConvLayer* L, int B, int H, int W) {
  if (!L->wp_bf16 || L->ks != 5 || conv_igemm_bf16_bn(L->cout, L->ks) != 128 || L->cout % 8) return false;
  ConvArgs a = conv_args(L, B, H, W);
  a.CoutP = L->coutp_bf16;
  return conv5_strip_bf16_supported(a, L->ks);
}

enum class DirectConv { KxfoldBf16, ThinBf16, IgemmBf16, ThinSplit16, ThinF32, SplitF32, IgemmF32 };
static DirectConv direct_route(const jcm_ctx* c, const ConvLayer* L, const ConvArgs& a, bool act_bf16, bool out_f32) {
  if (act_bf16) {
    if (L->thin_bf16 && out_f32) return L->wp_kxfold && conv_kxfold_bf16_supported(a, L->ks) ? DirectConv::KxfoldBf16 : DirectConv::ThinBf16;
    return DirectConv::IgemmBf16;
  }
  const bool use_split = L->wp_split && (L->thin ? c->f32_conv == 2 : conv_split_supported(L->ks, L->cin, L->coutp_split, a.B, a.H, a.W, c->split_min_wgs));
  if (L->thin) return use_split ? DirectConv::ThinSplit16 : DirectConv::ThinF32;
  return use_split ? DirectConv::SplitF32 : DirectConv::IgemmF32;
}
const char* conv_kernel_name(jcm_ctx* c, const ConvLayer* L, int B, int H, int W) {
  if (takes_fft(c, L, B, H, W)) return "conv_fft(cgemm_split_kernel)";
  const bool bf = c->precision == JCM_PRECISION_BF16;
  ConvArgs a = conv_args(L, B, H, W);
  a.relu_bn = L->has_bn ? 1 : 0;
  a.CoutP = bf ? L->coutp_bf16 : L->coutp;
  switch (direct_route(c, L, a, bf, L->thin_bf16)) {
    case DirectConv::KxfoldBf16: return "conv_kxfold_bf16_kernel";
    case DirectConv::ThinBf16: return "conv_thin_bf16_kernel";
    case DirectConv::ThinSplit16: return "conv_thin_split16_kernel";
    case DirectConv::ThinF32: return "conv_thin_f32_kernel";
    case DirectConv::SplitF32: return "conv_split_kernel";
    case DirectConv::IgemmF32: return "conv_igemm_f32_kernel";
    case DirectConv::IgemmBf16: break;
  }
  const int bn = conv_igemm_bf16_bn(L->cout, L->ks);
  return bn == 256 && conv_strip_bf16_supported(a, L->ks) ? "conv_strip_bf16_kernel"
         : L->ks == 5 && bn == 128 && conv5_strip_bf16_supported(a, L->ks) ? "conv5_strip_bf16_kernel" : "conv_igemm_bf16_kernel";
}

static int launch_conv_layer(jcm_ctx* c, const ConvLayer* L, const ConvCall& q) {
  ConvArgs a = conv_args(L, q.B, q.H, q.W);
  a.x = q.x; a.wp = q.act_bf16 ? L->wp_bf16 : static_cast<const void*>(L->wp); a.bias = L->bias; a.scale = L->scale; a.shift = L->shift; a.out = q.out;
  a.relu_bn = L->has_bn && !q.linear ? 1 : 0;
  a.in_planar = q.in_planar; a.out_planar = q.out_planar;
  a.hpool = q.hpool;
  a.CoutP = q.act_bf16 ? L->coutp_bf16 : L->coutp;
  if ((q.in_planar || q.out_planar) && !q.act_bf16) return fail(JCM_ERR_ARG, "planar activations exist on the bf16 path only");
  if (a.hpool && !q.act_bf16) return fail(JCM_ERR_STATE, "half pool requested on an fp32 layer");
  if (a.hpool && (q.out_f32 || L->thin_bf16 || L->ks != 5 || conv_igemm_bf16_bn(L->cout, L->ks) != 128 || !conv5_strip_bf16_supported(a, L->ks)))
    return fail(JCM_ERR_STATE, "half pool requested for a layer that does not run on conv5_strip_bf16_kernel");
  const DirectConv k = direct_route(c, L, a, q.act_bf16, q.out_f32);
  if (k == DirectConv::ThinSplit16 || k == DirectConv::SplitF32) {
    HIP_TRY(pow2_scale_of(static_cast<const float*>(q.x), (size_t)q.B * q.H * q.W * L->cin, c->act_scale, c->scale_scratch, c->stream));
    a.in_scale = c->act_scale;
    a.w_scale = L->wscale;
    a.wp = L->wp_split;
    a.CoutP = k == DirectConv::ThinSplit16 ? 16 : L->coutp_split;
  }
  switch (k) {
    case DirectConv::KxfoldBf16:
      a.wp = L->wp_kxfold;
      HIP_TRY(conv_kxfold_bf16(a, c->stream));
      break;
    case DirectConv::ThinBf16: HIP_TRY(conv_thin_bf16(a, c->stream)); break;
    case DirectConv::IgemmBf16: HIP_TRY(conv_igemm_bf16(a, L->ks, q.out_f32, c->stream)); break;
    case DirectConv::ThinSplit16: HIP_TRY(conv_thin_split16(a, c->stream)); break;
    case DirectConv::ThinF32: HIP_TRY(conv_thin_f32(a, c->stream)); break;
    case DirectConv::SplitF32: HIP_TRY(conv_split_f32(a, L->ks, 2, c->stream)); break;
    case DirectConv::IgemmF32: HIP_TRY(conv_igemm_f32(a, L->ks, c->stream)); break;
  }
  return JCM_OK;
}

bool takes_fft(jcm_ctx* c, const ConvLayer* L, int B, int H, int W) {
  if (!c->conv9_fft || c->f32_conv != 0 || (c->train && c->precision != JCM_PRECISION_F32) || (L->ks != 9 && L->ks != 5) || L->cin == 3 || !L->w_raw) return false;
  if (c->precision == JCM_PRECISION_BF16 && (L->ks != 9 || L->thin_bf16 || L->cout % 8)) return false;
  return conv_fft_supported(conv_args(L, B, H, W), L->ks);
}
enum class FftForm { Map, Win, Rows };
static std::string fft_cache_key(const std::string& scope, FftForm form, int H, int W) {
  return scope + (form == FftForm::Win ? "@win" : form == FftForm::Rows ? "@rows" : "@") + std::to_string(H) + "x" + std::to_string(W);
}
bool fft_spectra_valid(jcm_ctx* c, const std::string& scope, int H, int W, int circ) {
  auto it = c->fft_w.find(fft_cache_key(scope, circ ? FftForm::Win : FftForm::Map, H, W));
  return it != c->fft_w.end() && it->second.valid;
}
static const float* fft_forward_wscale(jcm_ctx* c, const std::string& scope, FftForm form, int H, int W) {
  static const std::string kDgrad = "dgrad:";
  if (scope.compare(0, kDgrad.size(), kDgrad) != 0) return nullptr;
  auto it = c->fft_w.find(fft_cache_key(scope.substr(kDgrad.size()), form, H, W));
  return it != c->fft_w.end() && it->second.valid ? it->second.wscale : nullptr;
}
void fft_cache_drop(jcm_ctx* c) {
  for (auto& kv : c->fft_w) (void)hipFree(kv.second.p);
  c->fft_w.clear();
}
void fft_cache_invalidate(jcm_ctx* c) {
  for (auto& kv : c->fft_w) kv.second.valid = false;
}
static int fft_cache_get(jcm_ctx* c, const std::string& scope, const std::string& key, size_t wbytes, jcm_ctx::FftW** out) {
  if (!c->fft_w.count(key)) {
    const size_t cap = (size_t)c->fft_cache_gb << 30;
    size_t held = 0;
    for (auto& kv : c->fft_w) held += kv.second.bytes;
    if (held + wbytes > cap && !c->fft_w.empty()) {
      JCM_TRY(sync_streams(c));
      fft_cache_drop(c);
    }
  }
  jcm_ctx::FftW& fw = c->fft_w[key];
  if (!fw.p) {
    const size_t wb = (wbytes + 255) & ~size_t(255);
    fw.bytes = wb + 256;
    if (hipMalloc(&fw.p, fw.bytes) != hipSuccess) {
      const size_t mb = fw.bytes >> 20;
      c->fft_w.erase(key);
      return fail(JCM_ERR_HIP, "out of device memory for the filter spectra of '" + scope + "' (" + std::to_string(mb) + " MB); jcm_set_option(\"conv9_fft\", 0) selects the direct kernels");
    }
    fw.wscale = reinterpret_cast<float*>(static_cast<char*>(fw.p) + wb);
  }
  *out = &fw;
  return JCM_OK;
}

int fft_new_words(jcm_ctx* c, int n, float** w) {
  if (n < 1) return fail(JCM_ERR_ARG, "fft_new_words: n < 1");
  for (;;) {
    if (c->fft_block_i < (int)c->fft_blocks.size()) {
      jcm_ctx::WordBlock& b = c->fft_blocks[c->fft_block_i];
      if (c->fft_word_i + n <= b.cap) {
        *w = b.p + c->fft_word_i;
        c->fft_word_i += n;
        return JCM_OK;
      }
      ++c->fft_block_i;
      c->fft_word_i = 0;
      continue;
    }
    jcm_ctx::WordBlock b;
    b.cap = n > jcm_ctx::kFftWords ? n : jcm_ctx::kFftWords;
    HIP_TRY(hipMalloc(reinterpret_cast<void**>(&b.p), (size_t)b.cap * sizeof(float)));
    if (hipError_t e = hipMemsetAsync(b.p, 0, (size_t)b.cap * sizeof(float), c->stream); e != hipSuccess) {
      (void)hipFree(b.p);
      return fail(JCM_ERR_HIP, std::string("hipMemsetAsync: ") + hipGetErrorString(e));
    }
    c->fft_blocks.push_back(b);
  }
}
int run_conv_fft(jcm_ctx* c, const ConvLayer* L, const std::string& scope, const ConvCall& q) {
  FftLink alone;
  FftLink& k = q.link ? *q.link : alone;
  const int B = q.B, H = q.H, W = q.W, circ = q.circ;
  const FftLayout in_layout = q.act_bf16 ? (q.in_planar ? kFftBf16Planar : kFftBf16Nhwc) : kFftF32Nhwc;
  const FftLayout out_layout = (q.act_bf16 && !q.out_f32) ? (q.out_planar ? kFftBf16Planar : kFftBf16Nhwc) : kFftF32Nhwc;
  FftArgs a = fft_args(L, B, H, W);
  a.x = q.x; a.bias = L->bias; a.scale = L->scale; a.shift = L->shift; a.out = q.out;
  a.CoutP = L->cout; a.relu_bn = L->has_bn && !q.linear ? 1 : 0;
  a.circ = circ;
  a.rows_mfma = c->fft_rows_mfma;
  a.fft_reg = c->fft_reg;
  a.win_map = k.win_map; a.win_scatter = k.win_scatter; a.win = k.win;
  const size_t mark = c->arena_off;
  const int np = fft_np(c);
  const int pool_ks = k.next.pool ? k.next.ks_next : 0;
  a.tiles = c->fft_tiles && k.next.pool ? 1 : 0;
  FftPlan plan = conv_fft_plan(a, L->ks, np, pool_ks);
  if (a.tiles && conv_fft_tiles_refusal(plan, in_layout, out_layout, k)) {
    a.tiles = 0;
    plan = conv_fft_plan(a, L->ks, np, pool_ks);
  }
  const int wH = a.tiles ? H / 2 : H, wW = a.tiles ? W / 2 : W;
  const int common = c->train ? 1 : 0;
  bool lrows = false;
  if (c->fft_logits_rows && k.t_in && !a.tiles) {
    const FftPlan lp = conv_fft_logits_plan(a);
    lrows = !conv_fft_logits_refusal(lp, L->ks, np, in_layout, out_layout, k, common);
    if (lrows) plan = lp;
  }
  void* work = arena_alloc<char>(c, plan.ok ? plan.total : 0);
  c->arena_off = mark;
  if (c->dry) return JCM_OK;
  const FftForm form = circ ? FftForm::Win : lrows ? FftForm::Rows : FftForm::Map;
  jcm_ctx::FftW* fwp = nullptr;
  JCM_TRY(fft_cache_get(c, scope, fft_cache_key(scope, form, wH, wW),
                        lrows ? conv_fft_logits_weight_bytes(wH, wW, L->cin) : conv_fft_weight_bytes(wH, wW, L->ks, L->cin, L->cout, np, circ), &fwp));
  jcm_ctx::FftW& fw = *fwp;
  if (!fw.valid) {
    if (lrows) HIP_TRY(conv_fft_logits_pack(L->w_raw, fw.p, wH, wW, L->cin, L->cout, c->stream, fw.wscale));
    else HIP_TRY(conv_fft_pack_weights(L->w_raw, fw.p, wH, wW, L->ks, L->cin, L->cout, np, c->precision == JCM_PRECISION_BF16, c->stream, fw.wscale, circ,
                                       np >= 4 ? fft_forward_wscale(c, scope, form, wH, wW) : nullptr));
    fw.valid = true;
  }
  plan.map.wp = plan.col.wp = plan.inv.wp = fw.p;
  hipEvent_t e0 = nullptr, e1 = nullptr, g0 = nullptr, g1 = nullptr;
  JCM_TRY(prof_begin(c, &e0, &e1));
  if (c->profile && (prof_event(c, &g0) != JCM_OK || prof_event(c, &g1) != JCM_OK)) { g0 = g1 = nullptr; }
  FftScale sc;
  if (np >= 4) {
    sc.tmax = k.tmax_in;
    if ((k.t_in || k.xs_ready) && !sc.tmax) return fail(JCM_ERR_STATE, "conv_fft '" + scope + "': a handed-over tensor without its scale word");
    if (!sc.tmax) JCM_TRY(fft_new_words(c, a.tiles ? 4 * B : B, &sc.tmax));
    if (k.t_next) JCM_TRY(fft_new_words(c, B, &sc.tmax_next));
    sc.winv = fw.wscale + 1;
    sc.common = common;
    sc.t16 = (np == kFftFp16x1 && c->fft_t16 && in_layout != kFftF32Nhwc && out_layout != kFftF32Nhwc && !k.xs && (!k.t_in || k.t_in_16) && (!k.t_next || (k.next.merge && !k.t_in))) ? 1 : 0;
  }
  k.tmax = sc.tmax;
  k.tmax_next = sc.tmax_next;
  const char* why = nullptr;
  const hipError_t e = lrows ? conv_fft_logits_f32(plan, L->ks, np, in_layout, out_layout, work, k, g0, g1, c->stream, &sc, &why)
                             : conv_fft_f32(plan, in_layout, out_layout, work, k, g0, g1, c->stream, np >= 4 ? &sc : nullptr, &why);
  if (g0 && g1 && e == hipSuccess) c->prof[scope + "/gemm"].emplace_back(g0, g1);
  else { if (g0) c->event_pool.push_back(g0); if (g1) c->event_pool.push_back(g1); }
  prof_end(c, scope, e0, e1, e == hipSuccess);
  if (e != hipSuccess) return fail(JCM_ERR_HIP, why ? "conv_fft '" + scope + "': " + why : std::string("conv_fft_f32: ") + hipGetErrorString(e));
  return JCM_OK;
}

int run_conv_layer(jcm_ctx* c, const ConvLayer* L, const std::string& scope, const ConvCall& q) {
  const bool fft = q.stride == 1 && takes_fft(c, L, q.B, q.H, q.W);
  if (q.linear && (q.act_bf16 || q.x_u8 || q.hpool || (q.link && !q.link->empty()))) return fail(JCM_ERR_STATE, "the linear epilogue of layer '" + scope + "' exists for a stand-alone fp32 layer only");
  if (!fft && q.link && !q.link->empty()) return fail(JCM_ERR_STATE, "layer '" + scope + "' was given a frequency-domain hand-over but does not run in the frequency domain");
  if (q.hpool && (fft || q.stride != 1)) return fail(JCM_ERR_STATE, "half pool requested for layer '" + scope + "', which does not run on conv5_strip_bf16_kernel");
  if (q.stride == 2) {
    if (c->dry) return JCM_OK;
    if (!(L->ks == 5 && L->cin == 3 && L->has_bn))
      return fail(JCM_ERR_ARG, "stride-2 kernel exists for 5x5, Cin=3, BN layers only (" + scope + ")");
    HIP_TRY(conv1_5x5s2(q.x, L->w_raw, L->bias, L->scale, L->shift, q.out, q.act_bf16, q.B, q.H, q.W, q.sub, L->cout, c->stream, q.x_u8, q.linear != 0));
    return JCM_OK;
  }
  if (fft) return run_conv_fft(c, L, scope, q);
  if (c->dry) return JCM_OK;
  if (q.stride != 1 || !(q.act_bf16 ? L->wp_bf16 : static_cast<const void*>(L->wp))) return fail(JCM_ERR_ARG, "no kernel for layer '" + scope + "' with stride " + std::to_string(q.stride));
  if (!q.act_bf16 && L->wp_stale) {
    HIP_TRY(pack_weights_f32(L->w_raw, L->wp, L->ks, L->cin, L->cout, L->coutp, c->stream));
    L->wp_stale = false;
  }
  hipEvent_t e0 = nullptr, e1 = nullptr;
  JCM_TRY(prof_begin(c, &e0, &e1));
  const int r = launch_conv_layer(c, L, q);
  prof_end(c, scope, e0, e1, r == JCM_OK);
  return r;
}
int run_conv(jcm_ctx* c, const std::string& scope, const ConvCall& q) {
  const ConvLayer* L = conv_of(c, scope);
  if (!L) return fail(JCM_ERR_STATE, "no conv layer '" + scope + "' (set '" + scope + "/weights' and finalize)");
  if (q.x_u8 && q.stride != 2) return fail(JCM_ERR_ARG, "byte images feed the stride-2 first layer only (" + scope + ")");
  return run_conv_layer(c, L, scope, q);
}

}
```

### joint-cnn-mrf_amd/csrc/ctx.h

```cpp
#pragma once
#include "../../include/jcm.h"

#include <map>
#include <mutex>
#include <string>
#include <vector>

#include "kernels.h"

namespace jcm {

struct CallOrder;

int fail(int code, const std::string& msg);

#define HIP_TRY(expr)                                                                                   \
  do {                                                                                                  \
    hipError_t e_ = (expr);                                                                             \
    if (e_ != hipSuccess)                                                                               \
      return ::jcm::fail(JCM_ERR_HIP, std::string(#expr) + ": " + hipGetErrorString(e_));               \
  } while (0)
#define JCM_TRY(expr)          \
  do {                         \
    int r_ = (expr);           \
    if (r_ != JCM_OK) return r_; \
  } while (0)
extern const char* const kJointNames[10];
constexpr int kC = 10;
constexpr float kBnEps = 1e-3f;
constexpr int kHmH = 60, kHmW = 90, kHmHW = kHmH * kHmW;
constexpr int kPrH = 120, kPrW = 180;
constexpr int kCH = 61, kCW = 91;
constexpr size_t kFrame = (size_t)kPrH * kPrW;
constexpr size_t kSpec = (size_t)kPrH * (kPrW / 2 + 1);

struct Tensor {
  std::vector<int64_t> shape;
  float* d = nullptr;
  size_t n = 0;
};

struct ConvLayer {
  int ks = 0, cin = 0, cout = 0, coutp = 0;
  bool has_bn = false;
  const float* w_raw = nullptr;
  float* wp = nullptr;
  mutable bool wp_stale = false;
  void* wp_split = nullptr;
  int coutp_split = 0;
  float* wscale = nullptr;
  void* wp_bf16 = nullptr;
  void* wp_kxfold = nullptr;
  void* wq1_bf16 = nullptr;
  float* wq1_f32 = nullptr;
  void* wq1_split = nullptr;
  int coutp_bf16 = 0;
  bool thin = false;
  bool thin_bf16 = false;
  const float* bias = nullptr;
  float* scale = nullptr;
  float* shift = nullptr;
};

struct TrainState;
}
struct jcm_ctx;
namespace jcm {
void train_destroy(jcm_ctx* c);
void dgrad_filters_stale(jcm_ctx* c);
const float* train_param_range(jcm_ctx* c, int64_t off, int64_t n);
const double* train_grad_sumsq(jcm_ctx* c);

}

struct jcm_ctx {
  int device = 0;
  hipStream_t stream = nullptr;
  int precision = JCM_PRECISION_F32;
  int K = 9;
  bool finalized = false;
  int f32_conv = 0;
  int split_min_wgs = 128;
  int sm_algo = 3;
  int conv9_fft = 1;
  int fft_tiles = 1;
  int fft_logits_rows = 1;
  int fft_fuse = 7;
  int fft_single = 1;
  int fft_t16 = 1;
  int fft_rows_mfma = 1;
  int fft_reg = 1;
  int fft_cache_gb = 64;
  int fft_win = 1;
  int bf16_hpool = 1;
  int torso_algo = 1;
  int sm_chunk = 32;
  int micro_batch = 0;
  int call_order = 1;
  int debug_skip = 0;
  std::map<std::string, jcm::Tensor> params;
  std::map<std::string, jcm::ConvLayer> convs;
  std::vector<void*> owned;
  size_t param_bytes = 0;
  bool has_sm = false;
  float* sp_energy = nullptr;
  float* sp_bias = nullptr;
  float* bn_sm_scale = nullptr;
  float* bn_sm_shift = nullptr;
  int* cond = nullptr;
  const float** energy_ptrs = nullptr;
  const float** bias_ptrs = nullptr;
  int* cond0 = nullptr;
  float2* prior_spec_t = nullptr;
  struct FftW { void* p = nullptr; size_t bytes = 0; bool valid = false; float* wscale = nullptr; };
  std::map<std::string, FftW> fft_w;
  double* hist_limits = nullptr;
  jcm::TrainState* train = nullptr;
  char* arena = nullptr;
  size_t arena_cap = 0, arena_off = 0, arena_peak = 0;
  bool dry = false;
  float* act_scale = nullptr;
  float* scale_scratch = nullptr;
  void* sm_scratch = nullptr;
  unsigned sm_epoch = 0;
  static constexpr int kFftWords = 1 << 18, kFftWordsPerCall = 1 << 16;
  struct WordBlock { float* p = nullptr; int cap = 0; };
  std::vector<WordBlock> fft_blocks;
  int fft_block_i = 0, fft_word_i = 0;
  struct Side {
    hipStream_t stream = nullptr;
    hipEvent_t fork = nullptr, join = nullptr;
    char* arena = nullptr;
    size_t arena_cap = 0, arena_off = 0, arena_peak = 0;
    std::vector<WordBlock> fft_blocks;
    int fft_block_i = 0, fft_word_i = 0;
    float* act_scale = nullptr;
    float* scale_scratch = nullptr;
  } side;
  int profile = 0;
  std::map<std::string, std::vector<std::pair<hipEvent_t, hipEvent_t>>> prof;
  std::vector<hipEvent_t> event_pool;
  std::mutex call_mu;
  int call_depth = 0;
  jcm::CallOrder* order = nullptr;
};

namespace jcm {

struct DeviceGuard {
  int prev = -1;
  explicit DeviceGuard(int dev) {
    (void)hipGetDevice(&prev);
    if (prev != dev) (void)hipSetDevice(dev);
    else prev = -1;
  }
  ~DeviceGuard() {
    if (prev >= 0) (void)hipSetDevice(prev);
  }
};

struct CallOrder {
  jcm_ctx* c;
  std::unique_lock<std::mutex> lk;
  std::unique_lock<std::mutex> hlk;
  bool nested = false;
  explicit CallOrder(jcm_ctx* ctx);
  ~CallOrder();
  void acquire();
  void release();
  CallOrder(const CallOrder&) = delete;
  CallOrder& operator=(const CallOrder&) = delete;
};

template <class T>
T* arena_alloc(jcm_ctx* c, size_t count) {
  const size_t bytes = (count * sizeof(T) + 255) & ~size_t(255);
  const size_t off = c->arena_off;
  c->arena_off += bytes;
  if (c->arena_off > c->arena_peak) c->arena_peak = c->arena_off;
  return reinterpret_cast<T*>(c->arena + off);
}

int arena_reserve(jcm_ctx* c, size_t bytes, size_t side_bytes);
int side_init(jcm_ctx* c);
int sync_streams(jcm_ctx* c);
int dev_alloc(jcm_ctx* c, void** p, size_t bytes);
int sm_scratch_next(jcm_ctx* c, void** scratch, unsigned* epoch);
const Tensor* find(jcm_ctx* c, const std::string& name);
int check(jcm_handle h, bool need_final);
const ConvLayer* conv_of(jcm_ctx* c, const std::string& scope);
int fold_bn(jcm_ctx* c, const std::string& scope, int n, float** scale, float** shift);
int refresh_derived(jcm_ctx* c, bool first);
int prof_event(jcm_ctx* c, hipEvent_t* e);
int prof_begin(jcm_ctx* c, hipEvent_t* e0, hipEvent_t* e1);
void prof_end(jcm_ctx* c, const std::string& scope, hipEvent_t e0, hipEvent_t e1, bool ok);
void prof_release_all(jcm_ctx* c, bool destroy);

inline ConvArgs conv_args(const ConvLayer* L, int B, int H, int W) {
  ConvArgs a{};
  a.B = B; a.H = H; a.W = W; a.Cin = L->cin; a.Cout = L->cout;
  return a;
}
inline FftArgs fft_args(const ConvLayer* L, int B, int H, int W) {
  FftArgs a{};
  static_cast<ConvArgs&>(a) = conv_args(L, B, H, W);
  return a;
}
struct ConvCall {
  const void* x = nullptr;
  void* out = nullptr;
  int B = 0, H = 0, W = 0;
  int stride = 1, sub = 1;
  bool act_bf16 = false;
  bool out_f32 = false;
  int in_planar = 0, out_planar = 0;
  bool x_u8 = false;
  FftLink* link = nullptr;
  int hpool = 0;
  int linear = 0;
  int circ = 0;
};
inline ConvCall conv_call(const void* x, void* out, int B, int H, int W) {
  ConvCall q;
  q.x = x; q.out = out; q.B = B; q.H = H; q.W = W;
  return q;
}
bool takes_fft(jcm_ctx* c, const ConvLayer* L, int B, int H, int W);
bool takes_strip(const ConvLayer* L, int B, int H, int W);
bool takes_c5strip(const ConvLayer* L, int B, int H, int W);
const char* conv_kernel_name(jcm_ctx* c, const ConvLayer* L, int B, int H, int W);
inline int fft_np(const jcm_ctx* c) { return c->precision == JCM_PRECISION_BF16 ? (c->fft_single ? 5 : 2) : 4; }
int fft_new_words(jcm_ctx* c, int n, float** w);
int run_conv_fft(jcm_ctx* c, const ConvLayer* L, const std::string& scope, const ConvCall& q);
int run_conv_layer(jcm_ctx* c, const ConvLayer* L, const std::string& scope, const ConvCall& q);
int run_conv(jcm_ctx* c, const std::string& scope, const ConvCall& q);
bool fft_spectra_valid(jcm_ctx* c, const std::string& scope, int H, int W, int circ = 0);
void fft_cache_drop(jcm_ctx* c);
void fft_cache_invalidate(jcm_ctx* c);

inline int cdiv2(int v) { return (v + 1) / 2; }

template <class S, class R>
int with_arena(jcm_ctx* c, S&& sizing, R&& real) {
  if (c->call_depth > 1) return fail(JCM_ERR_STATE, "this entry point uses the handle's workspace and cannot be called from the gradient-ready callback of the same handle");
  c->dry = true;
  c->arena_off = 0;
  c->arena_peak = 0;
  c->side.arena_peak = 0;
  int r = sizing();
  c->dry = false;
  if (r != JCM_OK) return r;
  JCM_TRY(arena_reserve(c, c->arena_peak, c->side.arena_peak));
  c->arena_off = 0;
  return real();
}
template <class F>
int with_arena(jcm_ctx* c, F&& body) {
  return with_arena(c, body, body);
}

bool conv1_pool_fused(const jcm_ctx* c, const ConvLayer* L1, int H, int W);
bool conv1_split_route(const jcm_ctx* c, const ConvLayer* L1);
int conv1_pool_stage(jcm_ctx* c, const std::string& scope, const ConvLayer* L1, const void* xin, bool xin_u8, int B, int xh, int xw, int xsub, void* dst, void** p1);
struct Pool2Layout {
  int pl23;
  int hp;
};
Pool2Layout pool2_layout(jcm_ctx* c, const ConvLayer* L2, const ConvLayer* L3, int B, int h2, int w2);
hipError_t pool2_launch(jcm_ctx* c, const Pool2Layout& l, const void* c2, void* p2, int B, int h2, int w2, int C);
int pd_forward_impl(jcm_ctx* c, const void* x, bool x_u8, int B, int H, int W, float* logits);
int sm_forward_impl(jcm_ctx* c, const float* hm, int Ca, const float* extra, int B, float* logits, int extra_ld = 0);

}
```

### joint-cnn-mrf_amd/csrc/fft_reg.h

```cpp
#pragma once
#include "fft_lds.h"

namespace jcm {
namespace fftr {
using namespace fftl;

constexpr double kPi = 3.14159265358979323846264338327950288;
constexpr double sin_small(double x) {
  double term = x, sum = x;
  for (int i = 1; i < 12; ++i) { term *= -x * x / ((2 * i) * (2 * i + 1)); sum += term; }
  return sum;
}
constexpr double cos_small(double x) {
  double term = 1.0, sum = 1.0;
  for (int i = 1; i < 12; ++i) { term *= -x * x / ((2 * i - 1) * (2 * i)); sum += term; }
  return sum;
}
struct SinCos { double s, c; };
constexpr SinCos sincos_frac(long num, long den) {
  num %= den;
  if (num < 0) num += den;
  const long n8 = num * 8;
  const long o = n8 / den;
  const double r = 2.0 * kPi * (double)(n8 - o * den) / (8.0 * (double)den);
  const double sr = sin_small(r), cr = cos_small(r), h = 0.70710678118654752440084436210485;
  switch (o) {
    case 0: return {sr, cr};
    case 1: return {h * (cr + sr), h * (cr - sr)};
    case 2: return {cr, -sr};
    case 3: return {h * (cr - sr), -h * (cr + sr)};
    case 4: return {-sr, -cr};
    case 5: return {-h * (cr + sr), -h * (cr - sr)};
    case 6: return {-cr, sr};
    default: return {-h * (cr - sr), h * (cr + sr)};
  }
}
template <int NUM, int DEN> struct Tw {
  static constexpr float re = (float)sincos_frac(NUM, DEN).c;
  static constexpr float im = (float)sincos_frac(NUM, DEN).s;
};
template <int NUM, int DEN> __device__ __forceinline__ cf twmul(cf a) {
  constexpr int n = ((NUM % DEN) + DEN) % DEN;
  if constexpr (n == 0) return a;
  else if constexpr (4 * n == DEN) return cf{-a.y, a.x};
  else if constexpr (2 * n == DEN) return cf{-a.x, -a.y};
  else if constexpr (4 * n == 3 * DEN) return cf{a.y, -a.x};
  else {
    constexpr float wr = Tw<n, DEN>::re, wi = Tw<n, DEN>::im;
    return cf{fmaf(-a.y, wi, a.x * wr), fmaf(a.x, wi, a.y * wr)};
  }
}

template <int N> struct RPlan;
template <> struct RPlan<96> { static constexpr int R1 = 8, R2 = 12; };
template <> struct RPlan<64> { static constexpr int R1 = 8, R2 = 8; };
template <> struct RPlan<48> { static constexpr int R1 = 4, R2 = 12; };
template <> struct RPlan<32> { static constexpr int R1 = 4, R2 = 8; };
template <> struct RPlan<16> { static constexpr int R1 = 4, R2 = 4; };
template <> struct RPlan<25> { static constexpr int R1 = 5, R2 = 5; };
template <> struct RPlan<14> { static constexpr int R1 = 2, R2 = 7; };
template <> struct RPlan<50> { static constexpr int R1 = 5, R2 = 10; };
template <> struct RPlan<36> { static constexpr int R1 = 3, R2 = 12; };
template <> struct RPlan<28> { static constexpr int R1 = 4, R2 = 7; };
template <> struct RPlan<20> { static constexpr int R1 = 4, R2 = 5; };

template <int N, int S, int N2, int K1 = 0>
__device__ __forceinline__ void step1_twiddle(cf (&x)[N], const cf (&a)[RPlan<N>::R1]) {
  constexpr int R1 = RPlan<N>::R1, R2 = RPlan<N>::R2;
  x[R2 * K1 + N2] = twmul<S * N2 * K1, N>(a[K1]);
  if constexpr (K1 + 1 < R1) step1_twiddle<N, S, N2, K1 + 1>(x, a);
}
template <int N, int S, int N2 = 0>
__device__ __forceinline__ void step1(cf (&x)[N]) {
  constexpr int R1 = RPlan<N>::R1, R2 = RPlan<N>::R2;
  cf a[R1];
#pragma unroll
  for (int n1 = 0; n1 < R1; ++n1) a[n1] = x[R2 * n1 + N2];
  Dft<R1, S>::run(a);
  step1_twiddle<N, S, N2>(x, a);
  if constexpr (N2 + 1 < R2) step1<N, S, N2 + 1>(x);
}
template <int N, int S, int K1>
__device__ __forceinline__ void step2_row(const cf (&x)[N], cf (&out)[RPlan<N>::R2]) {
  constexpr int R2 = RPlan<N>::R2;
#pragma unroll
  for (int n2 = 0; n2 < R2; ++n2) out[n2] = x[R2 * K1 + n2];
  Dft<R2, S>::run(out);
}

}
}
```

### joint-cnn-mrf_amd/csrc/kernels.h

```cpp
#pragma once
#include <hip/hip_runtime.h>
#include <stdint.h>

#include <atomic>

namespace jcm {

struct LdsAttr {
  std::atomic<uint64_t> done{0};
  hipError_t ensure(const void* fn, int bytes) {
    int dev = 0;
    hipError_t e = hipGetDevice(&dev);
    if (e != hipSuccess) return e;
    const uint64_t bit = 1ull << (dev & 63);
    if (done.load(std::memory_order_acquire) & bit) return hipSuccess;
    e = hipFuncSetAttribute(fn, hipFuncAttributeMaxDynamicSharedMemorySize, bytes);
    if (e == hipSuccess) done.fetch_or(bit, std::memory_order_release);
    return e;
  }
};

struct ConvArgs {
  const void* x;
  const void* wp;
  const float* bias;
  const float* scale;
  const float* shift;
  void* out;
  int B, H, W, Cin, Cout, CoutP;
  int relu_bn;
  const float* in_scale = nullptr;
  const float* w_scale = nullptr;
  int in_planar = 0, out_planar = 0;
  int hpool = 0;
};
int conv_igemm_bn(int Cout);
hipError_t conv_igemm_f32(const ConvArgs& a, int ks, hipStream_t st);
hipError_t pack_weights_f32(const float* w_hwio, float* wp, int ks, int Cin, int Cout, int CoutP, hipStream_t st);

bool conv_split_supported(int ks, int Cin, int CoutP, int B, int H, int W, int min_wgs);
size_t conv_split_weight_bytes(int ks, int Cin, int CoutP, int ns);
hipError_t pack_weights_split(const float* w_hwio, void* wp, int ks, int Cin, int Cout, int CoutP, int ns, hipStream_t st,
                              const float* w_scale = nullptr);
hipError_t conv_split_f32(const ConvArgs& a, int ks, int ns, hipStream_t st);

hipError_t conv_thin_split16(const ConvArgs& a, hipStream_t st);

hipError_t conv_thin_f32(const ConvArgs& a, hipStream_t st);

hipError_t conv_thin_bf16(const ConvArgs& a, hipStream_t st);

enum FftOperand : int { kFftBf16x2 = 2, kFftFp16x2 = 4, kFftFp16x1 = 5 };
enum FftLayout : int { kFftF32Nhwc = 0, kFftBf16Nhwc = 1, kFftBf16Planar = 2 };
struct FftScale {
  float* tmax = nullptr;
  float* tmax_next = nullptr;
  const float* winv = nullptr;
  int common = 0;
  int t16 = 0;
};
struct Fp16Scale {
  float* tmax = nullptr;
  float* tmax_next = nullptr;
  const float* winv = nullptr;
  float hf = 0.f;
  int nb = 0;
  int common = 0;
  int t16 = 0;
  float* t16_fwd = nullptr;
  float* t16_inv = nullptr;
  int t16_cb = 64;
};
struct WinGeom {
  int B = 0, H = 0, W = 0, TY = 0, TX = 0;
  int BW() const { return B * TY * TX; }
};
struct FftArgs : ConvArgs {
  int circ = 0;
  const void* win_map = nullptr;
  int win_valid_only = 0;
  bool win_scatter = false;
  WinGeom win;
  int tiles = 0;
  int rows_mfma = 0;
  int fft_reg = 1;
};
bool conv_fft_supported(const ConvArgs& a, int ks, int circ = 0);
size_t conv_fft_weight_bytes(int H, int W, int ks, int Cin, int Cout, int np, int circ = 0);
hipError_t conv_fft_pack_weights(const float* w_hwio, void* wf, int H, int W, int ks, int Cin, int Cout, int np, bool round_bf16, hipStream_t st,
                                 float* wscale = nullptr, int circ = 0,
                                 const float* bound_from = nullptr);
size_t conv_fft_workspace_bytes(const FftArgs& a, int ks, int np);
struct FftMerge { const void* x2; int H2, W2; const void* x3; int H3, W3; };
struct FftNext { int pool = 0; int ks_next = 0; const FftMerge* merge = nullptr; };
struct FftLink {
  const void* t_in = nullptr;
  bool t_in_16 = false;
  float* tmax_in = nullptr;
  const FftMerge* merge = nullptr;
  void* xs = nullptr;
  bool xs_ready = false;
  const void* win_map = nullptr;
  WinGeom win;
  void* t_next = nullptr;
  FftNext next;
  bool win_scatter = false;
  float* tmax = nullptr;
  float* tmax_next = nullptr;
  bool empty() const { return !t_in && !merge && !xs && !xs_ready && !win_map && !t_next && !next.pool && !next.merge && !win_scatter; }
};
size_t conv_fft_logits_weight_bytes(int H, int W, int Cin);
hipError_t conv_fft_logits_pack(const float* w_hwio, void* aop, int H, int W, int Cin, int Cout, hipStream_t st, float* wscale);
bool conv_fft_win_gather_supported(int win, int Cin, bool fft_reg);
bool conv_fft_win_scatter_supported(int win, int Cout, bool fft_reg);
bool conv_fft_pool_fusable(const ConvArgs& a, int ks, int ks_next);
size_t conv_fft_pool_handover_bytes(const ConvArgs& a, int ks_next);
bool conv_fft_merge_fusable(const ConvArgs& a, int ks, int ks_next, const FftMerge& m, bool fft_reg, bool h16 = false);
size_t conv_fft_xs_bytes(const FftArgs& a, int ks, int np);
hipError_t conv_fft_spectra(const FftArgs& a, int ks, int np, void* work, void* xs, hipStream_t st, float* tmax = nullptr, int common = 0, const char** why = nullptr);
bool conv_fft_geometry(int H, int W, int ks, int B, int Cout, int np, int* NY, int* NX, int* MT, int circ = 0);

size_t wgrad_fft_scratch_bytes(int NY, int NX, int Cin, int Cout);
hipError_t wgrad_fft(const void* xs, const void* zs, void* scratch, const float* w, float lmbd, float* dw, int ks, int NY, int NX, int B, int MTx, int MTz, int Cin,
                     int ldz, int Cout, hipStream_t st, int np = 3, const float* tmax_x = nullptr, const float* tmax_z = nullptr, int H = 0);
hipError_t pad_channels_f32(const float* in, int ldi, float* out, int ldo, size_t N, hipStream_t st);
hipError_t window_gather_f32(const float* map, float* win, int B, int H, int W, int C, int WS, int TY, int TX, int valid_only, hipStream_t st);
hipError_t window_scatter_f32(const float* val, float* map, int B, int H, int W, int C, int WS, int TY, int TX, hipStream_t st);
bool conv_fft_fusable(const ConvArgs& a, int ks, int ks_next);
size_t conv_fft_handover_bytes(const ConvArgs& a, int ks, bool h16 = false);

int cgemm_split_mtile(int np, int B, int Cout);
int cgemm_split_ntile(int np, int Cout);
int cgemm_split_parts(int np);
size_t cgemm_split_w_bytes(int np, int F, int Cin, int Cout);
float cgemm_split_y16_shift(int Cin);
hipError_t cgemm_split(const void* xs, const void* ws, void* y, int np, int F, int B, int Cin, int Cout, int ldy, hipStream_t st, float y16_shift = 0.f);

bool conv5_strip_bf16_supported(const ConvArgs& a, int ks);
hipError_t conv5_strip_bf16(const ConvArgs& a, hipStream_t st);

bool conv_kxfold_bf16_supported(const ConvArgs& a, int ks);
size_t conv_kxfold_weight_bytes(int Cin);
hipError_t pack_weights_kxfold(const float* w_hwio, void* wp, int Cin, hipStream_t st);
hipError_t conv_kxfold_bf16(const ConvArgs& a, hipStream_t st);

int conv_igemm_bf16_bn(int Cout, int ks);
hipError_t conv_igemm_bf16(const ConvArgs& a, int ks, bool out_f32, hipStream_t st);
hipError_t pack_weights_bf16(const float* w_hwio, void* wp, int ks, int Cin, int Cout, int CoutP, hipStream_t st);

bool conv_strip_bf16_supported(const ConvArgs& a, int ks);
hipError_t conv_strip_bf16(const ConvArgs& a, hipStream_t st);

hipError_t conv1_5x5s2(const void* x, const float* w, const float* bias, const float* scale, const float* shift,
                       void* out, bool out_bf16, int B, int H0, int W0, int sub, int Cout, hipStream_t st, bool x_u8 = false,
                       bool linear = false);

hipError_t pack_conv1_bf16(const float* w_hwio, void* wq, hipStream_t st);
hipError_t conv1_mfma_pool(const void* x, const void* wq, const float* bias, const float* scale, const float* shift,
                           void* out, int B, int H0, int W0, int sub, hipStream_t st, bool x_u8 = false);

hipError_t pack_conv1_f32(const float* w_hwio, float* wq, hipStream_t st);
size_t conv1_split_weight_bytes();
hipError_t pack_conv1_split(const float* w_hwio, void* wq, hipStream_t st);
hipError_t conv1_mfma_pool_split(const void* x, const void* wq, const float* bias, const float* scale, const float* shift, float* out,
                                 int B, int H0, int W0, int sub, hipStream_t st, bool x_u8 = false);
hipError_t conv1_mfma_pool_f32(const void* x, const float* wq, const float* bias, const float* scale, const float* shift, float* out,
                               int B, int H0, int W0, int sub, hipStream_t st, bool x_u8 = false);

hipError_t max_pool_2x2(const void* x, void* out, bool bf16, int B, int H, int W, int C, hipStream_t st);
hipError_t vpool_2x1_bf16(const void* x, void* out, int B, int H, int W, int C, hipStream_t st);
hipError_t planar_to_nhwc_bf16(const void* x, void* out, int B, int HW, int C, hipStream_t st);
hipError_t resize_bilinear(const float* x, float* out, int B, int H, int W, int C, int OH, int OW, hipStream_t st);
hipError_t upsample_merge3(const void* x1, const void* x2, int H2, int W2, const void* x3, int H3, int W3,
                           void* out, bool bf16, int B, int H, int W, int C, hipStream_t st);
hipError_t upsample_merge3_planar(const void* x1, const void* x2, int H2, int W2, const void* x3, int H3, int W3,
                                  void* out, int B, int H, int W, int C, hipStream_t st);
hipError_t spatial_softmax(const float* in, float* out, int B, int HW, int K, hipStream_t st);
hipError_t argmax_coords(const float* hm, int32_t* coords, int B, int HW, int WW, int K, hipStream_t st);
hipError_t softmax_argmax(const float* logits, float* prob, int32_t* coords, int B, int HW, int WW, int K, hipStream_t st);

hipError_t det_curve(const int32_t* pred, const float* y, int B, int HW, int WW, int K, int C, const float* radii, int R, int32_t* true_out, float* nd_out,
                     int32_t* hits, hipStream_t st);
hipError_t hm_peaks(const float* hm, int B, int HH, int WW, int K, int P, float threshold, int32_t* cells, float* offsets, float* scores, int32_t* count,
                    hipStream_t st);
constexpr int kPoseMaxB = 1 << 20;
hipError_t pose_decode(const float* hm10, int B, const int32_t* cells, const int32_t* count, int P, const float* sp_energy, const float* sp_bias,
                       const float* bn_scale, const float* bn_shift, float* V, float* M, float* pscore, int32_t* ppose, int32_t* index, int32_t* coords,
                       float* score, float* score0, hipStream_t st);
constexpr int kTorsoMaxB = 1 << 20;
hipError_t torso_infer_direct(const float* prob, int B, const float* sp_energy, const float* bn_scale, const float* bn_shift, float* lik, float* corr,
                              float* energy, int32_t* cell, float* torso, hipStream_t st);
hipError_t torso_blobs(const int32_t* cells_in, int B, float* torso, hipStream_t st);
hipError_t mirror_pairs(const void* x, bool x_u8, int B, int H, int W, int C, void* out, hipStream_t st);
hipError_t mirror_merge(const float* hm, int n, int G, int HH, int WW, int K, const int* perm, float* out, hipStream_t st);
constexpr int kFitMax = 64;
constexpr int kFitTW = 32;
struct FitBatch {
  int64_t off[kFitMax];
  int h[kFitMax], w[kFitMax];
  int first[kFitMax + 1];
};
struct FitGeom {
  int y0, x0, ch, cw;
};
__host__ __device__ inline FitGeom fit_geometry(int h, int w, int OH, int OW) {
  FitGeom g;
  if ((int64_t)OH * w <= (int64_t)OW * h) {
    g.ch = OH;
    const int64_t cw = (2 * (int64_t)w * OH + h) / (2 * (int64_t)h);
    g.cw = cw < 1 ? 1 : (int)cw;
  } else {
    g.cw = OW;
    const int64_t ch = (2 * (int64_t)h * OW + w) / (2 * (int64_t)w);
    g.ch = ch < 1 ? 1 : (int)ch;
  }
  g.y0 = (OH - g.ch) / 2;
  g.x0 = (OW - g.cw) / 2;
  return g;
}
hipError_t fit_images(const uint8_t* src, int64_t src_bytes, const int64_t* desc, int B, int C, int OH, int OW, int pad, bool out_f32, void* out,
                      hipStream_t st);
constexpr int kFitWinMax = 64;
struct FitWinBatch {
  int64_t off[kFitWinMax];
  int h[kFitWinMax], w[kFitWinMax];
  int wy0[kFitWinMax], wx0[kFitWinMax], wh[kFitWinMax], ww[kFitWinMax];
  int first[kFitWinMax + 1];
};
hipError_t fit_windows(const uint8_t* src, int64_t src_bytes, const int64_t* desc, int NW, int C, int OH, int OW, int pad, bool out_f32, void* out,
                       hipStream_t st);
constexpr int kRenderMax = 64;
constexpr int kRenderTile = 8192;
constexpr int kRenderPrimMax = 256;
struct RenderBatch {
  int64_t off[kRenderMax];
  int h[kRenderMax], w[kRenderMax];
  int first[kRenderMax + 1];
  int pfirst[kRenderMax + 1];
  int gy0[kRenderMax], gx0[kRenderMax], gch[kRenderMax], gcw[kRenderMax];
};
struct RenderHeat {
  const float* hm;
  const float* maxima;
  int hh, hw, K, stride, gain;
  uint8_t mask[16];
};
size_t render_prim_ints(int NP);
hipError_t render_poses(const uint8_t* src, const int64_t* desc, int B, uint8_t* out, const int32_t* prims, int NP, int32_t* prims_dev,
                        const float* hm, int hh, int hw, int K, int stride, const int32_t* geom, const uint8_t* heat_mask, int heat_gain,
                        float* maxima, hipStream_t st);
constexpr int kSynthRecInts = 20;
constexpr int kSynthPrimInts = 16;
constexpr int kSynthPrimMax = 64;
constexpr int kSynthTile = 8192;
hipError_t synth_people(const int32_t* records, int B, const int32_t* prims, int NP, int H, int W, bool out_f32, void* out, int32_t* records_dev,
                        int32_t* prims_dev, hipStream_t st);
constexpr int kSeqMaxHW = 8192;
constexpr int kSeqMaxK = 16;
constexpr int kSeqMaxR = 16;
hipError_t seq_put_taps(const double* taps_host, int n, double* taps_dev, hipStream_t st);
hipError_t seq_filter(const float* hm, int S, int T, int HH, int WW, int K, const double* taps, int R, double om, double u, const int32_t* shift,
                      const double* state_in, float* filtered, int32_t* coords, double* norm, int32_t* reset, double* state_out, hipStream_t st);
hipError_t seq_viterbi(const float* hm, int S, int T, int HH, int WW, int K, const double* taps, int R, double om, double u, const int32_t* shift,
                       int16_t* bp, int32_t* amax, int32_t* path, double* maxes, int32_t* breaks, hipStream_t st);
constexpr int kSeqSmoothMaxHW = 6144;
hipError_t seq_smooth(const float* hm, int S, int T, int HH, int WW, int K, const double* taps, int R, double om, double u, double* belief, float* smoothed,
                      int32_t* coords, float* conf, double* norm, int32_t* reset, double* mass, int32_t* cut, double* trans, hipStream_t st);
hipError_t seq_smooth_lag(const float* hm, int S, int W, int P, int E, int L, int HH, int WW, int K, const double* taps, int R, double om, double u,
                          int32_t* scan_coords, double* belief, double* norm, int32_t* reset, float* smoothed, int32_t* coords, float* conf, double* mass,
                          int32_t* cut, hipStream_t st);
hipError_t seq_tracks_filter(const float* hm, int S, int T, int HH, int WW, int M, const double* taps, int R, double om, double u, int D,
                             const double* state_in, float* filtered, int32_t* coords, double* norm, int32_t* reset, double* state_out, float* value,
                             hipStream_t st);
hipError_t seq_tracks_viterbi(const float* hm, int S, int T, int HH, int WW, int M, const double* taps, int R, double om, double u, int D, int16_t* bp,
                              int32_t* amax, int32_t* path, double* maxes, int32_t* breaks, float* value, hipStream_t st);
constexpr int kFrameShiftMaxD = 16;
constexpr int kFrameShiftMaxSide = 4096;
constexpr int kFrameShiftMaxT = 65534;
size_t frame_shift_slots(int pairs, int D);
hipError_t frame_shift(const uint8_t* x, int T, int H, int W, int y0, int x0, int ch, int cw, int D, const uint8_t* prev, uint16_t* L, uint16_t* C,
                       unsigned long long* slots, int32_t* center, int32_t* disp, int64_t* sad, hipStream_t st);
hipError_t bn_fold(const float* gamma, const float* beta, const float* mean, const float* var, float eps, float* scale, float* shift,
                   int n, hipStream_t st);

hipError_t sm_softplus5(const float* in, float* out, int64_t n, hipStream_t st);
hipError_t sm_softplus5_multi(const float* const* in, float* out, int P, int64_t n, hipStream_t st);
hipError_t sm_likelihood(const float* hm, int Ca, const float* extra, const float* bn_scale, const float* bn_shift, float* lik,
                         int B, int C, hipStream_t st, int extra_ld = 0);
hipError_t sm_pair_conv(const float* priors, const float* maps, const int* cond, float* cpre,
                        int B, int P, int C, hipStream_t st);
hipError_t sm_finish(const float* lik, const float* cpre, const float* spbias, float* logits,
                     int B, int K, int C, hipStream_t st);
hipError_t sm_resize_only(const float* cpre, float* out, int B, hipStream_t st);

hipError_t sm_pad_frame(const float* hm, int Ca, const float* extra, const float* sc, const float* sh, float* frame, int B, int C,
                        hipStream_t st, int extra_ld = 0);
hipError_t sm_spec_mul(const float2* lhat, const float2* phat, const int* cond, float2* spec, int B, int C, int P, hipStream_t st);
hipError_t sm_resize_frame(const float* cfull, float* out, int B, hipStream_t st);
hipError_t sm_fused_forward(const float* hm, int Ca, const float* extra, int extra_ld, const float* sc, const float* sh, const float2* phat_t,
                            const int* cond, const float* spbias, float2* lhat_t, float* logits, int B, int K, int C, hipStream_t st,
                            float* tsave, void* scratch, unsigned epoch);
size_t sm_fused_scratch_bytes();
hipError_t sm_fused_spectra(const float* hm, int Ca, const float* extra, int extra_ld, const float* sc, const float* sh, float2* lhat_t, int B, int C,
                            hipStream_t st);
hipError_t sm_lds_fwd_frames(const float* frames, float2* spec_t, int n, hipStream_t st);
hipError_t sm_lds_fwd_dframes(const float* G, const float* T, float2* dhat_t, int nb, int K, int P, hipStream_t st);
hipError_t sm_lds_inv_frames(const float2* spec_t, float* frames, int n, int r0, int nrows, float scale, hipStream_t st);

hipError_t window_resize(const float* src, int H, int W, int C, const int* windows_dev, int NW, float2* mm_scratch,
                         int OH, int OW, float* out, hipStream_t st);
hipError_t group_mean(const float* in, float* out, int n, int G, size_t M, hipStream_t st);

size_t augment_scratch_doubles(int B);
hipError_t augment_train(const float* x, const float* y, const float* params, int B, int H, int W, int hh, int hw, double* scratch,
                         float* x_out, float* y_out, hipStream_t st);

constexpr int kGatherMax = 256;
struct GatherIdx {
  int v[kGatherMax];
};
hipError_t gather_batch(const float* x_all, const float* y_all, const int* idx, int B, size_t nx, size_t ny, float* x_out, float* y_out,
                        hipStream_t st);
hipError_t gather_batch_u8(const uint8_t* x_all, const float* y_all, const int* idx, int B, size_t nx, size_t ny, float* x_out, float* y_out,
                           hipStream_t st);
hipError_t u8_to_f32_array(const uint8_t* x, float* x_out, size_t n, hipStream_t st);
hipError_t augment_train_indexed(const float* x_all, const float* y_all, const int* idx, const float* params, int B, int H, int W, int hh, int hw,
                                 double* scratch, float* x_out, float* y_out, hipStream_t st);
hipError_t augment_train_indexed_u8(const uint8_t* x_all, const float* y_all, const int* idx, const float* params, int B, int H, int W, int hh, int hw,
                                    double* scratch, float* x_out, float* y_out, hipStream_t st);

size_t train_reduce_scratch_doubles(int C);
hipError_t bn_batch_stats(const void* x, bool bf16, size_t N, int C, float eps, float decay, float* mean, float* rstd, float* mov_mean,
                          float* mov_var, double* scratch, hipStream_t st);
hipError_t bn_apply(const void* r, const float* mean, const float* rstd, const float* gamma, const float* beta, void* y, bool bf16, size_t N,
                    int C, hipStream_t st);
hipError_t bn_bwd_reduce(const void* dy, float dy_scale, const void* r, bool bf16, const float* mean, const float* rstd, size_t N, int C,
                         float* sums, float* dgamma, float* dbeta, double* scratch, hipStream_t st);
hipError_t bn_bwd_apply(const void* dy, float dy_scale, const void* r, bool bf16, const float* mean, const float* rstd, const float* gamma,
                        const float* sums, size_t N, int C, int relu, void* dz, hipStream_t st);
hipError_t col_sum(const void* x, bool bf16, size_t N, int C, float* out, double* scratch, hipStream_t st);
bool bn_apply_pool(const void* r, const float* mean, const float* rstd, const float* gamma, const float* beta, void* y, void* p, bool bf16, int B, int H, int W, int C,
                   hipStream_t st);
bool bn_bwd_pooled(const void* dp, const void* y, const void* r, bool bf16, const float* mean, const float* rstd, const float* gamma, int B, int H, int W, int C, float* sums,
                   float* dgamma, float* dbeta, void* dz, float* colsum, double* scratch, hipStream_t st, hipError_t* err);
hipError_t bn_bwd_apply_colsum(const void* dy, float dy_scale, const void* r, bool bf16, const float* mean, const float* rstd, const float* gamma, const float* sums, size_t N,
                               int C, int relu, void* dz, float* colsum, double* scratch, hipStream_t st);
hipError_t max_pool_bwd(const void* x, const void* dy, void* dx, bool bf16, int B, int H, int W, int C, hipStream_t st);
hipError_t cast_pad_bf16(const float* in, int ldi, void* out, int ldo, size_t N, hipStream_t st);
hipError_t cast_bf16_f32(const void* in, float* out, size_t n, hipStream_t st);
hipError_t resize_bilinear_bwd(const void* dy, void* dx, bool bf16, int B, int h, int w, int H, int W, int C, float scale, hipStream_t st);
hipError_t softmax_ce(const float* logits, const float* target, int B, int HW, int K, int Kt, float gscale, float* loss, float* dz,
                      int ldz, int accumulate, hipStream_t st);
hipError_t softmax_bwd(const float* p, const float* g, int B, int HW, int K, int ldg, float* dz, int ldz, hipStream_t st);
hipError_t loss_means_accumulate(const float* ce, int n, float scale, float* out, bool first, hipStream_t st);
hipError_t sum_squares(const float* x, size_t n, double* out, int accumulate, double* scratch, hipStream_t st);
hipError_t sum_squares_chunks(float* const* w, const int64_t* start, const int* len, const int* flag, int nchunks, double* out, double* scratch, hipStream_t st);
hipError_t adam_update(float* w, const float* g, float* m, float* v, size_t n, const double* sumsq, float clip, float lr_t, float b1,
                       float b2, float eps, hipStream_t st);
hipError_t momentum_update(float* w, const float* g, float* acc, size_t n, const double* sumsq, float clip, float lr, float mom,
                           hipStream_t st);
hipError_t scale_copy(const float* a, float s, float* out, size_t n, hipStream_t st);
hipError_t optimizer_chunks(float* const* wptr, const int64_t* cstart, const int64_t* coff, const int* clen, int nchunks, const float* g,
                            float* m, float* v, const double* sumsq, float clip, float lr_t, float b1, float b2, float eps, int momentum_mode,
                            hipStream_t st);

int wgrad_splits(int ks, int Cin, int Cout, int B, int H);
hipError_t wgrad_f32(const float* x, const float* dz, float* partial, int splits, int ks, int B, int H, int W, int Cin, int Cout, int ldz,
                     hipStream_t st);
hipError_t wgrad_reduce(const float* partial, int splits, size_t n, const float* w, float lmbd, float* dw, hipStream_t st, const float* out_scale = nullptr);
int wgrad_conv1_blocks(void);
hipError_t wgrad_reduce_wide(const float* partial, int splits, size_t n, const float* w, float lmbd, float* dw, hipStream_t st);
hipError_t wgrad_conv1(const float* x, const void* dz, bool dz_bf16, float* partial, int B, int H0, int W0, int sub, int Cout, hipStream_t st);
hipError_t split_parts16(const float* x, void* out_f16_2n, size_t n, const float* scale, hipStream_t st);
hipError_t pow2_scale_of(const float* x, size_t n, float* scale, float* scratch, hipStream_t st);
hipError_t wgrad_split16(const void* xp, const void* zp, float* partial, int splits, int ks, int B, int H, int W, int Cin, int Cout, int ldz,
                         hipStream_t st);
bool wgrad_split_supported(int ks, int Cin, int ldz);
hipError_t wgrad_bf16(const void* x, const void* dz, float* partial, int splits, int ks, int B, int H, int W, int Cin, int Cout, int ldz,
                      hipStream_t st);
hipError_t flip_transpose_weights(const float* w_hwio, float* wd, int ks, int Cin, int Cout, int CoP, hipStream_t st);

hipError_t bn_fold_stats(const float* mean, const float* rstd, const float* gamma, const float* beta, float* sc, float* sh, int n,
                         hipStream_t st);
hipError_t sm_concat_target(const float* prob, const float* y, float* out, size_t N, int K, int C, hipStream_t st);
hipError_t sm_bwd_dbias(const float* G, const float* T, float* dspb, int nb, int K, int P, int accumulate, hipStream_t st);
hipError_t sm_bwd_spec_da(const float2* Dhat, const float2* Lhat, const int* cond, float2* dA, int nb, int C, int P, int accumulate,
                          hipStream_t st);
hipError_t sm_bwd_spec_dl(const float2* Dhat, const float2* Ahat, float2* dL, int nb, int K, int C, hipStream_t st);
hipError_t sm_bwd_dh(const float* dLframe, const float* G, const float* frame, const float* hm, const float* sc, const float* sh, float* dh,
                     int nb, int K, int C, hipStream_t st);
hipError_t sm_bwd_params(const float* dAframe, const float* dspb, const float* const* e_ptr, const float* const* b_ptr, const int64_t* e_off,
                         const int64_t* b_off, float* grads, int P, hipStream_t st);

}
```

### joint-cnn-mrf_amd/csrc/options.h

```cpp
#pragma once
#include <climits>

#include "ctx.h"

namespace jcm {

struct Option {
  enum Kind { BOOL, RANGE, EITHER };
  const char* name;
  int jcm_ctx::*field;
  Kind kind;
  int64_t lo, hi;
  bool before_finalize;
  const char* env;
  int (*on_change)(jcm_ctx*, int64_t);
};

int option_profile(jcm_ctx* c, int64_t value);
int option_fft_single(jcm_ctx* c, int64_t value);

inline constexpr Option kOptions[] = {
    {"precision",       &jcm_ctx::precision,       Option::RANGE,  0,  1,       true,  nullptr,               nullptr},
    {"n_joints",        &jcm_ctx::K,               Option::RANGE,  1,  9,       true,  nullptr,               nullptr},
    {"f32_conv",        &jcm_ctx::f32_conv,        Option::EITHER, 0,  2,       true,  nullptr,               nullptr},
    {"split_min_wgs",   &jcm_ctx::split_min_wgs,   Option::RANGE,  0,  INT_MAX, false, nullptr,               nullptr},
    {"profile",         &jcm_ctx::profile,         Option::BOOL,   0,  1,       false, nullptr,               option_profile},
    {"conv9_fft",       &jcm_ctx::conv9_fft,       Option::BOOL,   0,  1,       false, nullptr,               nullptr},
    {"call_order",      &jcm_ctx::call_order,      Option::BOOL,   0,  1,       false, nullptr,               nullptr},
    {"fft_single",      &jcm_ctx::fft_single,      Option::BOOL,   0,  1,       false, nullptr,               option_fft_single},
    {"fft_t16",         &jcm_ctx::fft_t16,         Option::BOOL,   0,  1,       false, nullptr,               nullptr},
    {"fft_rows_mfma",   &jcm_ctx::fft_rows_mfma,   Option::BOOL,   0,  1,       false, nullptr,               nullptr},
    {"fft_windows",     &jcm_ctx::fft_win,         Option::BOOL,   0,  1,       false, nullptr,               nullptr},
    {"fft_fuse",        &jcm_ctx::fft_fuse,        Option::RANGE,  0,  7,       false, nullptr,               nullptr},
    {"fft_tiles",       &jcm_ctx::fft_tiles,       Option::BOOL,   0,  1,       false, "JCM_FFT_TILES",       nullptr},
    {"fft_logits_rows", &jcm_ctx::fft_logits_rows, Option::BOOL,   0,  1,       false, "JCM_FFT_LOGITS_ROWS", nullptr},
    {"fft_reg",         &jcm_ctx::fft_reg,         Option::BOOL,   0,  1,       false, "JCM_FFT_REG",         nullptr},
    {"fft_cache_gb",    &jcm_ctx::fft_cache_gb,    Option::RANGE,  0,  1 << 20, false, "JCM_FFT_CACHE_GB",    nullptr},
    {"bf16_hpool",      &jcm_ctx::bf16_hpool,      Option::BOOL,   0,  1,       false, nullptr,               nullptr},
    {"sm_algo",         &jcm_ctx::sm_algo,         Option::EITHER, 1,  3,       false, nullptr,               nullptr},
    {"torso_algo",      &jcm_ctx::torso_algo,      Option::EITHER, 1,  1,       false, nullptr,               nullptr},
    {"sm_chunk",        &jcm_ctx::sm_chunk,        Option::RANGE,  1,  INT_MAX, false, nullptr,               nullptr},
    {"micro_batch",     &jcm_ctx::micro_batch,     Option::RANGE,  0,  INT_MAX, false, nullptr,               nullptr},
    {"debug_skip",      &jcm_ctx::debug_skip,      Option::RANGE,  0,  127,     false, nullptr,               nullptr},
};

}
```

Before: 7757 images/sec.

## Split 60-row 9x9 FFT convolutions into two overlapping 30-row y windows

Adds a y-window form for 9x9 FFT convolutions on 60-row maps. Each image is cut into two overlapping 38-row windows, which are transformed with a 40-point column FFT instead of a longer one, run through the channel GEMM as 2B rows, and scattered back into the full row buffer before the inverse row pass. It is meant to shrink the transform length and spectra size where the GEMM cost dominates, as judged by a cost heuristic. In exchange it doubles the GEMM batch, adds halo work and new kernel variants, and is enabled by default.

After: 7803 images/sec (median of 6 runs). Within noise of the previous version (+0.6%).

```diff
diff --git a/joint-cnn-mrf_amd/csrc/conv_fft.hip b/joint-cnn-mrf_amd/csrc/conv_fft.hip
--- a/joint-cnn-mrf_amd/csrc/conv_fft.hip
+++ b/joint-cnn-mrf_amd/csrc/conv_fft.hip
@@ -321,7 +321,7 @@
 FftPlan conv_fft_plan(const FftArgs& a, int ks, int np, int pool_ks_next) {
   FftPlan p;
   Sizes s, n;
-  p.ok = a.tiles ? sizes_of(a.H / 2, a.W / 2, ks, &s) : sizes_of(a.H, a.W, ks, &s, a.circ);
+  p.ok = a.tiles ? sizes_of(a.H / 2, a.W / 2, ks, &s) : a.ywin ? sizes_of(kYwinSpectraH, a.W, ks, &s) : sizes_of(a.H, a.W, ks, &s, a.circ);
   if (!p.ok) return p;
   p.ks = ks; p.np = np;
   p.NY = s.NY; p.NX = s.NX; p.NXH = s.NX / 2 + 1; p.F = s.NY * p.NXH;
@@ -332,8 +332,10 @@
   p.map.CoutP = pad64(a.Cout);
   p.col = p.map;
   if (a.tiles) { p.col.B = 4 * a.B; p.col.H = s.NY; p.col.W = a.W / 2; p.col.tiles = 0; }
+  if (a.ywin) { p.col.B = 2 * a.B; p.col.H = kYwinHeld; }
   p.inv = p.col;
   if (a.tiles) p.inv.H = a.H / 2;
+  if (a.ywin) p.inv.H = kYwinValid;
   if (a.circ) { p.inv.H = a.H - 8; p.inv.W = a.W - 8; }
   const FftArgs& c = p.col;
   p.ldy = padn(c.Cout, cgemm_split_ntile(np, c.Cout));
@@ -342,7 +344,8 @@
   p.inv_cb = s.NY > 100 ? 32 : 64;
   const size_t cop = pad64(c.Cout), cmax = (size_t)c.Cin > cop ? c.Cin : cop;
   const size_t bp = (size_t)(c.B + p.MT - 1) / p.MT * p.MT;
-  carve(&p, (size_t)c.B * p.NXH * c.H * cmax * sizeof(cf), (size_t)p.F * bp * c.Cin * 4 * cgemm_split_parts(np), (size_t)p.F * c.B * p.ldy * sizeof(cf),
+  const size_t trows = a.ywin ? (size_t)a.B * a.H : (size_t)c.B * c.H;
+  carve(&p, trows * p.NXH * cmax * sizeof(cf), (size_t)p.F * bp * c.Cin * 4 * cgemm_split_parts(np), (size_t)p.F * c.B * p.ldy * sizeof(cf),
         (size_t)c.B * c.H * (c.Cin / CB) * sizeof(float), (size_t)c.B * p.NXH * (cop / p.inv_cb) * sizeof(float));
   return p;
 }
@@ -415,6 +418,18 @@
   if (a.H % 4 || a.W % 4 || !p.ok || !cfft_tiles_supported(p.NY, p.NX, a)) return "tiles exist for the model's 120 x 180 map geometry";
   return nullptr;
 }
+const char* conv_fft_ywin_refusal(const FftPlan& p, FftLayout in, FftLayout out, const FftLink& k) {
+  const FftArgs& a = p.map;
+  if (!a.ywin) return "not planned as y windows";
+  if (const char* no = conv_fft_refusal(p, in, out, k, 0)) return no;
+  if (p.np != kFftFp16x2 || in != kFftF32Nhwc || out != kFftF32Nhwc) return "y windows exist on fp32 handles (operand form 4, fp32 NHWC on both sides)";
+  if (a.circ || a.tiles || a.win_map || a.win_scatter || k.win_map || k.win_scatter || k.xs || k.xs_ready) return "y windows take whole maps and keep no spectra";
+  if (!a.fft_reg) return "y windows exist with the register kernels only";
+  if (p.ks != 9 || a.H != 2 * kYwinValid || p.NY != 40 || p.NX != 96) return "y windows exist for 9x9 layers on 60-row maps with 96-point rows";
+  if (a.Cout % CB) return "y windows take output channels in whole blocks of 64";
+  if (p.col.B > p.MT) return "y windows need the 2 B rows of the channel GEMM in one M tile";
+  return nullptr;
+}
 const char* conv_fft_logits_refusal(const FftPlan& p, int ks, int np, FftLayout in, FftLayout out, const FftLink& k, int common) {
   const FftArgs& a = p.map;
   if (ks != 9 || np != kFftFp16x2 || in != kFftF32Nhwc || out != kFftF32Nhwc) return "logits rows: a 9x9 layer of an fp32 handle, fp32 NHWC on both sides";
@@ -442,7 +457,7 @@
   if (p.np < 4 || !in) return sc;
   sc.tmax = in->tmax; sc.tmax_next = in->tmax_next; sc.winv = in->winv; sc.common = in->common; sc.t16 = in->t16;
   sc.hf = hf;
-  sc.nb = p.col.B;
+  sc.nb = p.map.ywin ? p.map.B : p.col.B;
   if (sc.t16) {
     sc.t16_fwd = p.at<float>(work, p.t16_fwd);
     sc.t16_inv = p.at<float>(work, p.t16_inv);
@@ -467,7 +482,10 @@
   if (a.win_map) return cfft_rows_fwd_win_reg(p.NX, a, r.T, r.sc.tmax, r.st);
   return (r.reg() && cfft_rows_fwd_reg(p.NX, a, in, r.T, r.sc.tmax, r.st, r.sc.t16_fwd)) || cfft_rows_fwd(p.NX, a, in, r.T, p.twx, r.sc.tmax, r.st, r.sc.t16_fwd);
 }
-bool pass_cols_fwd(const Run& r, const cf* Tin) { return cfft_cols_fwd(r.p.NY, r.p.col, r.p.np, Tin, r.Xs, r.p.twy, r.p.NXH, r.p.MT, r.sc, r.st); }
+bool pass_cols_fwd(const Run& r, const cf* Tin) {
+  if (r.p.map.ywin) return cfft_cols_fwd_ywin(r.p.NY, r.p.col, r.p.map.H, kYwinValid, Tin, r.Xs, r.p.twy, r.p.NXH, r.p.MT, r.sc, r.st);
+  return cfft_cols_fwd(r.p.NY, r.p.col, r.p.np, Tin, r.Xs, r.p.twy, r.p.NXH, r.p.MT, r.sc, r.st);
+}
 hipError_t pass_gemm(const Run& r, hipEvent_t g0, hipEvent_t g1) {
   const FftArgs& c = r.p.col;
   if (g0 && hipEventRecord(g0, r.st) != hipSuccess) return hipErrorUnknown;
@@ -477,6 +495,7 @@
 }
 bool pass_cols_inv(const Run& r) {
   const FftPlan& p = r.p;
+  if (p.map.ywin) return r.reg() && cfft_cols_inv_reg(p.NY, p.inv, r.Yf, r.T, p.NXH, p.ldy, p.opad + 4, r.st, nullptr, 0.f);
   if (r.reg() && p.inv_cb == 64 && cfft_cols_inv_reg(p.NY, p.inv, r.Yf, r.T, p.NXH, p.ldy, p.opad, r.st, r.sc.t16_inv, r.yinv)) return true;
   if (p.map.tiles) return false;
   return cfft_cols_inv(p.NY, p.inv, r.Yf, r.T, p.twy, p.NXH, p.ldy, p.opad, r.st, r.sc.t16_inv, r.yinv);
@@ -493,10 +512,11 @@
     return (r.reg() && cfft_rows_inv_merge_fwd_reg(p.NX, a, *k.next.merge, r.T, Tn, p.opad, p.norm, r.sc, r.st)) || cfft_rows_inv_merge_fwd(p.NX, a, *k.next.merge, r.T, Tn, p.twx, p.opad, p.norm, r.sc, r.st);
   }
   if (Tn) return (r.reg() && cfft_rows_inv_fwd_reg(p.NX, a, r.T, Tn, p.opad, p.norm, r.sc, r.st)) || cfft_rows_inv_fwd(p.NX, a, r.T, Tn, p.twx, p.opad, p.norm, r.sc, r.st);
-  if ((p.inv.rows_mfma & 1) && cfft_rows_inv_mfma(p.NX, p.inv, out, r.T, p.opad, p.norm, r.sc, r.st)) return true;
-  if (r.reg() && cfft_rows_inv_reg(p.NX, p.inv, out, r.T, p.opad, p.norm, r.sc, r.st)) return true;
-  if (p.inv.win_scatter) return false;
-  return cfft_rows_inv(p.NX, p.inv, out, r.T, p.twx, p.opad, p.norm, r.sc, r.st);
+  const FftArgs& ri = a.ywin ? a : p.inv;
+  if ((ri.rows_mfma & 1) && cfft_rows_inv_mfma(p.NX, ri, out, r.T, p.opad, p.norm, r.sc, r.st)) return true;
+  if (r.reg() && cfft_rows_inv_reg(p.NX, ri, out, r.T, p.opad, p.norm, r.sc, r.st)) return true;
+  if (ri.win_scatter) return false;
+  return cfft_rows_inv(p.NX, ri, out, r.T, p.twx, p.opad, p.norm, r.sc, r.st);
 }
 const char* scale_refusal(const FftPlan& p, const FftScale* sc, const FftLink& k) {
   if (p.np < 4) return nullptr;
@@ -508,7 +528,7 @@
 
 hipError_t conv_fft_f32(FftPlan p, FftLayout in, FftLayout out, void* work, const FftLink& k, hipEvent_t g0, hipEvent_t g1, hipStream_t st, const FftScale* scp, const char** why) {
   const int t16 = p.np >= 4 && scp ? scp->t16 : 0;
-  if (const char* no = p.map.tiles ? conv_fft_tiles_refusal(p, in, out, k) : conv_fft_refusal(p, in, out, k, t16)) return refuse(why, no);
+  if (const char* no = p.map.tiles ? conv_fft_tiles_refusal(p, in, out, k) : p.map.ywin ? conv_fft_ywin_refusal(p, in, out, k) : conv_fft_refusal(p, in, out, k, t16)) return refuse(why, no);
   if (const char* no = scale_refusal(p, scp, k)) return refuse(why, no);
   if (hipError_t e = conv_fft_plan_twiddles(&p); e != hipSuccess) return e;
   Run r{p, p.at<cf>(work, p.T), k.xs ? k.xs : p.at<void>(work, p.Xs), p.at<cf>(work, p.Yf), device_scale(p, scp, (float)p.col.H, work), 0.f, 0.f, st};
diff --git a/joint-cnn-mrf_amd/csrc/conv_fft_cols.hip b/joint-cnn-mrf_amd/csrc/conv_fft_cols.hip
--- a/joint-cnn-mrf_amd/csrc/conv_fft_cols.hip
+++ b/joint-cnn-mrf_amd/csrc/conv_fft_cols.hip
@@ -3,9 +3,11 @@
 namespace jcm {
 namespace cfft {
 
-template <int NY, int NP, bool T16 = false>
+template <int NY, int NP, bool T16 = false, bool YWIN = false>
 __global__ __launch_bounds__(colfwd_threads<NY>()) void cols_fwd_split_kernel(const cf* __restrict__ T, uint4* __restrict__ Xs, const cf* __restrict__ twg, int B, int H, int KC, int MT,
-                                                            int mtiles, const float* __restrict__ tmax, int common, const float* __restrict__ t16, int ntiles) {
+                                                            int mtiles, const float* __restrict__ tmax, int common, const float* __restrict__ t16, int ntiles,
+                                                            int BI, int HM, int HV) {
+  static_assert(!YWIN || (NP == 4 && !T16), "the y windows exist on fp32 handles");
   constexpr int IMG = colimg<NY>(), CH = IMG * 16, NTC = colfwd_threads<NY>(), NPP = NP == 5 ? 1 : 2;
   constexpr int CPV = T16 ? 4 : 2;
   constexpr int NV = NY * CH / CPV, KV = (NV + NTC - 1) / NTC, VPR = CH / CPV, VPI = 16 / CPV;
@@ -31,6 +33,13 @@
 #pragma unroll
     for (int i = 0; i < KV; ++i) {
       const int t = tid + i * NTC, y = t / VPR, v = t % VPR, img = v / VPI, cv = v % VPI;
+      if constexpr (YWIN) {
+        const int m = b0 + img, w = m >= BI ? 1 : 0, ym = y + w * HV - 4;
+        const bool ok = t < NV && y < H && img < nimg && ym >= 0 && ym < HM;
+        const uint4* map = reinterpret_cast<const uint4*>(T) + ((size_t)kx * KC + kc) * BI * HM * VPI;
+        pre[i] = ok ? map[((size_t)(m - w * BI) * HM + ym) * VPI + cv] : make_uint4(0u, 0u, 0u, 0u);
+        continue;
+      }
       const bool ok = t < NV && y < H && img < nimg;
       pre[i] = ok ? src[((size_t)img * H + y) * VPI + cv] : make_uint4(0u, 0u, 0u, 0u);
       if constexpr (T16) psc[i] = ok ? t16[((size_t)(b0 + img) * (KC >> 2) + (kc >> 2)) * H + y] : 0.f;
@@ -55,7 +64,10 @@
       }
     }
     if constexpr (NP >= 4)
-      if (tid < IMG) xsc[tid] = tid < nimg ? fp16_scale(tmax_of(tmax, b0 + tid, B, common), (float)H) : 1.f;
+      if (tid < IMG) {
+        const int m = b0 + tid;
+        xsc[tid] = tid >= nimg ? 1.f : YWIN ? fp16_scale(tmax_of(tmax, m >= BI ? m - BI : m, BI, common), (float)H) : fp16_scale(tmax_of(tmax, m, B, common), (float)H);
+      }
     __syncthreads();
     if (tile + (int)gridDim.x < ntiles) prefetch(tile + (int)gridDim.x);
     fft<NY, -1, CH, NTC>(buf, tw, tid);
@@ -157,7 +169,7 @@
   do {                                                                                                           \
     if (ATTR.ensure(reinterpret_cast<const void*>(KERNEL), lds) != hipSuccess) return false;                      \
     const dim3 grid((unsigned)persistent_grid(reinterpret_cast<const void*>(KERNEL), ntiles, (int)blk.x, lds));  \
-    hipLaunchKernelGGL(KERNEL, grid, blk, lds, st, T, static_cast<uint4*>(Xs), tw, a.B, a.H, KC, MT, mtiles, __VA_ARGS__, ntiles); \
+    hipLaunchKernelGGL(KERNEL, grid, blk, lds, st, T, static_cast<uint4*>(Xs), tw, a.B, a.H, KC, MT, mtiles, __VA_ARGS__, ntiles, 0, 0, 0); \
   } while (0)
   if (np == 5 && sc.t16_fwd) {
     if (!sc.tmax || (KC & 3)) return false;
@@ -188,6 +200,18 @@
 #undef CALL
   return e;
 }
+bool cfft_cols_fwd_ywin(int NY, const FftArgs& col, int HM, int HV, const cf* T, void* Xs, const cf* tw, int NXH, int MT, const Fp16Scale& sc, hipStream_t st) {
+  constexpr int N = 40, IMG = colimg<N>(), lds = (N * IMG * 16 + N) * (int)sizeof(cf);
+  if (NY != N || !col.ywin || (col.B & 1) || col.B > MT || col.H > N || HV + 8 != col.H || HM != 2 * HV || !sc.tmax || sc.t16_fwd) return false;
+  const int KC = col.Cin / 16, ntiles = NXH * KC * ((col.B + IMG - 1) / IMG);
+  static LdsAttr attr;
+  const void* kernel = reinterpret_cast<const void*>(cols_fwd_split_kernel<N, 4, false, true>);
+  if (attr.ensure(kernel, lds) != hipSuccess) return false;
+  const dim3 grid((unsigned)persistent_grid(kernel, ntiles, colfwd_threads<N>(), lds)), blk(colfwd_threads<N>());
+  hipLaunchKernelGGL((cols_fwd_split_kernel<N, 4, false, true>), grid, blk, lds, st, T, static_cast<uint4*>(Xs), tw, col.B, col.H, KC, MT, 1, sc.tmax, sc.common, (const float*)nullptr, ntiles,
+                     col.B / 2, HM, HV);
+  return true;
+}
 bool cfft_cols_inv(int NY, const FftArgs& a, const cf* Yf, cf* T, const cf* tw, int NXH, int ldy, int pad, hipStream_t st, float* t16, float y16_inv) {
 #define CALL(N) launch_cols_inv<N>(a, Yf, T, tw, NXH, ldy, pad, st, t16, y16_inv)
   CFFT_BY_SIZE(NY, CALL)
diff --git a/joint-cnn-mrf_amd/csrc/conv_fft_common.h b/joint-cnn-mrf_amd/csrc/conv_fft_common.h
--- a/joint-cnn-mrf_amd/csrc/conv_fft_common.h
+++ b/joint-cnn-mrf_amd/csrc/conv_fft_common.h
@@ -263,6 +263,7 @@
 bool cfft_rows_fwd(int NX, const FftArgs& a, FftLayout layout, cf* T, const cf* tw, float* tmax, hipStream_t st, float* t16 = nullptr);
 bool cfft_rows_fwd_merge(int NX, const FftArgs& a, const FftMerge& m, FftLayout in_layout, cf* T, const cf* tw, float* tmax, hipStream_t st, float* t16 = nullptr);
 bool cfft_cols_fwd(int NY, const FftArgs& a, int np, const cf* T, void* Xs, const cf* tw, int NXH, int MT, const Fp16Scale& sc, hipStream_t st);
+bool cfft_cols_fwd_ywin(int NY, const FftArgs& col, int HM, int HV, const cf* T, void* Xs, const cf* tw, int NXH, int MT, const Fp16Scale& sc, hipStream_t st);
 bool cfft_cols_inv(int NY, const FftArgs& a, const cf* Yf, cf* T, const cf* tw, int NXH, int ldy, int pad, hipStream_t st, float* t16 = nullptr, float y16_inv = 0.f);
 bool cfft_rows_inv(int NX, const FftArgs& a, FftLayout layout, const cf* T, const cf* tw, int pad, float norm, const Fp16Scale& sc, hipStream_t st);
 bool cfft_rows_inv_fwd(int NX, const FftArgs& a, const cf* T, cf* Tn, const cf* tw, int pad, float norm, const Fp16Scale& sc, hipStream_t st);
diff --git a/joint-cnn-mrf_amd/csrc/conv_fft_plan.h b/joint-cnn-mrf_amd/csrc/conv_fft_plan.h
--- a/joint-cnn-mrf_amd/csrc/conv_fft_plan.h
+++ b/joint-cnn-mrf_amd/csrc/conv_fft_plan.h
@@ -37,6 +37,10 @@
 
 const char* conv_fft_refusal(const FftPlan& p, FftLayout in, FftLayout out, const FftLink& link, int t16);
 const char* conv_fft_tiles_refusal(const FftPlan& p, FftLayout in, FftLayout out, const FftLink& link);
+constexpr int kYwinValid = 30, kYwinHeld = kYwinValid + 8;
+constexpr int kYwinSpectraH = kYwinValid + 4;
+const char* conv_fft_ywin_refusal(const FftPlan& p, FftLayout in, FftLayout out, const FftLink& link);
+inline bool conv_fft_ywin_pays(int B, int Cin, int Cout) { return (long long)1176 * Cin * Cout > (long long)2 * 784 * B * (Cin + Cout); }
 const char* conv_fft_logits_refusal(const FftPlan& p, int ks, int np, FftLayout in, FftLayout out, const FftLink& link, int common);
 
 hipError_t conv_fft_f32(FftPlan p, FftLayout in, FftLayout out, void* work, const FftLink& link, hipEvent_t g0, hipEvent_t g1, hipStream_t st, const FftScale* sc,
diff --git a/joint-cnn-mrf_amd/csrc/conv_fft_reg_inv.hip b/joint-cnn-mrf_amd/csrc/conv_fft_reg_inv.hip
--- a/joint-cnn-mrf_amd/csrc/conv_fft_reg_inv.hip
+++ b/joint-cnn-mrf_amd/csrc/conv_fft_reg_inv.hip
@@ -72,16 +72,22 @@
   }
 }
 
-template <int NY, bool T16>
+template <int NY, bool T16, bool YWIN = false>
 __global__ __launch_bounds__(256) __attribute__((amdgpu_waves_per_eu(NY >= 64 ? 2 : 3, NY >= 64 ? 2 : 8))) void cols_inv_reg_kernel(const cf* __restrict__ Yf, void* __restrict__ T, int B, int H, int NXH, int C, int ldy,
-                                                                                              int pad, float* __restrict__ t16, float yinv) {
+                                                                                              int pad, float* __restrict__ t16, float yinv, int BI) {
   static_assert(NY % 2 == 0, "ky pairs");
+  static_assert(!(YWIN && T16), "the y windows exist on fp32 handles");
   constexpr int R1 = RPlan<NY>::R1, R2 = RPlan<NY>::R2;
   const size_t g = (size_t)blockIdx.x * 256 + threadIdx.x;
   const int c = (int)(g % C);
   const unsigned bk = (unsigned)__builtin_amdgcn_readfirstlane((int)(g / C));
   const int kx = (int)(bk % (unsigned)NXH), b = (int)(bk / (unsigned)NXH);
   if (b >= B) return;
+  int row0 = b * H;
+  if constexpr (YWIN) {
+    const int w = b / BI;
+    row0 = ((b - w * BI) * 2 + w) * H;
+  }
   const bool odd = (c & 1) != 0;
   cf x[NY];
   if constexpr (T16) {
@@ -127,7 +133,7 @@
 #pragma unroll
     for (int i = 0; i < NY; ++i) {
       const int y = (i / R2) + R1 * (i % R2) - pad;
-      if (y >= 0 && y < H) st_stream(reinterpret_cast<cf*>(T) + ((size_t)(b * H + y) * NXH + kx) * C + c, x[i]);
+      if (y >= 0 && y < H) st_stream(reinterpret_cast<cf*>(T) + ((size_t)(row0 + y) * NXH + kx) * C + c, x[i]);
     }
   }
 }
@@ -135,10 +141,15 @@
   if (a.CoutP % 64 || ((y16_inv != 0.f) != (t16 != nullptr)) || (t16 && ldy % 2)) return false;
   const size_t threads = (size_t)a.B * NXH * a.CoutP;
   const dim3 grid((unsigned)((threads + 255) / 256)), blk(256);
+  if (a.ywin) {
+    if (NY != 40 || t16 || (a.B & 1) || pad + a.H > NY) return false;
+    hipLaunchKernelGGL((cols_inv_reg_kernel<40, false, true>), grid, blk, 0, st, Yf, static_cast<void*>(T), a.B, a.H, NXH, a.CoutP, ldy, pad, nullptr, 0.f, a.B / 2);
+    return true;
+  }
 #define CI_LAUNCH(N)                                                                                                                                             \
   do {                                                                                                                                                           \
-    if (t16) hipLaunchKernelGGL((cols_inv_reg_kernel<N, true>), grid, blk, 0, st, Yf, static_cast<void*>(T), a.B, a.H, NXH, a.CoutP, ldy, pad, t16, y16_inv);            \
-    else hipLaunchKernelGGL((cols_inv_reg_kernel<N, false>), grid, blk, 0, st, Yf, static_cast<void*>(T), a.B, a.H, NXH, a.CoutP, ldy, pad, nullptr, 0.f);          \
+    if (t16) hipLaunchKernelGGL((cols_inv_reg_kernel<N, true>), grid, blk, 0, st, Yf, static_cast<void*>(T), a.B, a.H, NXH, a.CoutP, ldy, pad, t16, y16_inv, 0);         \
+    else hipLaunchKernelGGL((cols_inv_reg_kernel<N, false>), grid, blk, 0, st, Yf, static_cast<void*>(T), a.B, a.H, NXH, a.CoutP, ldy, pad, nullptr, 0.f, 0);       \
   } while (0)
   switch (NY) {
     case 64: CI_LAUNCH(64); break;
diff --git a/joint-cnn-mrf_amd/csrc/conv_route.hip b/joint-cnn-mrf_amd/csrc/conv_route.hip
--- a/joint-cnn-mrf_amd/csrc/conv_route.hip
+++ b/joint-cnn-mrf_amd/csrc/conv_route.hip
@@ -89,9 +89,9 @@
   if (c->precision == JCM_PRECISION_BF16 && (L->ks != 9 || L->thin_bf16 || L->cout % 8)) return false;
   return conv_fft_supported(conv_args(L, B, H, W), L->ks);
 }
-enum class FftForm { Map, Win, Rows };
+enum class FftForm { Map, Win, Rows, YWin };
 static std::string fft_cache_key(const std::string& scope, FftForm form, int H, int W) {
-  return scope + (form == FftForm::Win ? "@win" : form == FftForm::Rows ? "@rows" : "@") + std::to_string(H) + "x" + std::to_string(W);
+  return scope + (form == FftForm::Win ? "@win" : form == FftForm::Rows ? "@rows" : form == FftForm::YWin ? "@ywin" : "@") + std::to_string(H) + "x" + std::to_string(W);
 }
 bool fft_spectra_valid(jcm_ctx* c, const std::string& scope, int H, int W, int circ) {
   auto it = c->fft_w.find(fft_cache_key(scope, circ ? FftForm::Win : FftForm::Map, H, W));
@@ -181,7 +181,13 @@
     a.tiles = 0;
     plan = conv_fft_plan(a, L->ks, np, pool_ks);
   }
-  const int wH = a.tiles ? H / 2 : H, wW = a.tiles ? W / 2 : W;
+  if (c->fft_ywin && !c->train && !a.tiles && !circ && L->ks == 9 && conv_fft_ywin_pays(B, L->cin, L->cout)) {
+    a.ywin = 1;
+    const FftPlan wp = conv_fft_plan(a, L->ks, np, pool_ks);
+    if (conv_fft_ywin_refusal(wp, in_layout, out_layout, k)) a.ywin = 0;
+    else plan = wp;
+  }
+  const int wH = a.tiles ? H / 2 : a.ywin ? kYwinSpectraH : H, wW = a.tiles ? W / 2 : W;
   const int common = c->train ? 1 : 0;
   bool lrows = false;
   if (c->fft_logits_rows && k.t_in && !a.tiles) {
@@ -192,9 +198,9 @@
   void* work = arena_alloc<char>(c, plan.ok ? plan.total : 0);
   c->arena_off = mark;
   if (c->dry) return JCM_OK;
-  const FftForm form = circ ? FftForm::Win : lrows ? FftForm::Rows : FftForm::Map;
+  const FftForm form = circ ? FftForm::Win : lrows ? FftForm::Rows : a.ywin ? FftForm::YWin : FftForm::Map;
   jcm_ctx::FftW* fwp = nullptr;
-  JCM_TRY(fft_cache_get(c, scope, fft_cache_key(scope, form, wH, wW),
+  JCM_TRY(fft_cache_get(c, scope, a.ywin ? fft_cache_key(scope, form, H, W) : fft_cache_key(scope, form, wH, wW),
                         lrows ? conv_fft_logits_weight_bytes(wH, wW, L->cin) : conv_fft_weight_bytes(wH, wW, L->ks, L->cin, L->cout, np, circ), &fwp));
   jcm_ctx::FftW& fw = *fwp;
   if (!fw.valid) {
diff --git a/joint-cnn-mrf_amd/csrc/ctx.h b/joint-cnn-mrf_amd/csrc/ctx.h
--- a/joint-cnn-mrf_amd/csrc/ctx.h
+++ b/joint-cnn-mrf_amd/csrc/ctx.h
@@ -84,6 +84,7 @@
   int sm_algo = 3;
   int conv9_fft = 1;
   int fft_tiles = 1;
+  int fft_ywin = 1;
   int fft_logits_rows = 1;
   int fft_fuse = 7;
   int fft_single = 1;
diff --git a/joint-cnn-mrf_amd/csrc/fft_reg.h b/joint-cnn-mrf_amd/csrc/fft_reg.h
--- a/joint-cnn-mrf_amd/csrc/fft_reg.h
+++ b/joint-cnn-mrf_amd/csrc/fft_reg.h
@@ -60,6 +60,7 @@
 template <> struct RPlan<25> { static constexpr int R1 = 5, R2 = 5; };
 template <> struct RPlan<14> { static constexpr int R1 = 2, R2 = 7; };
 template <> struct RPlan<50> { static constexpr int R1 = 5, R2 = 10; };
+template <> struct RPlan<40> { static constexpr int R1 = 8, R2 = 5; };
 template <> struct RPlan<36> { static constexpr int R1 = 3, R2 = 12; };
 template <> struct RPlan<28> { static constexpr int R1 = 4, R2 = 7; };
 template <> struct RPlan<20> { static constexpr int R1 = 4, R2 = 5; };
diff --git a/joint-cnn-mrf_amd/csrc/kernels.h b/joint-cnn-mrf_amd/csrc/kernels.h
--- a/joint-cnn-mrf_amd/csrc/kernels.h
+++ b/joint-cnn-mrf_amd/csrc/kernels.h
@@ -82,6 +82,7 @@
   bool win_scatter = false;
   WinGeom win;
   int tiles = 0;
+  int ywin = 0;
   int rows_mfma = 0;
   int fft_reg = 1;
 };
diff --git a/joint-cnn-mrf_amd/csrc/options.h b/joint-cnn-mrf_amd/csrc/options.h
--- a/joint-cnn-mrf_amd/csrc/options.h
+++ b/joint-cnn-mrf_amd/csrc/options.h
@@ -33,6 +33,7 @@
     {"fft_windows",     &jcm_ctx::fft_win,         Option::BOOL,   0,  1,       false, nullptr,               nullptr},
     {"fft_fuse",        &jcm_ctx::fft_fuse,        Option::RANGE,  0,  7,       false, nullptr,               nullptr},
     {"fft_tiles",       &jcm_ctx::fft_tiles,       Option::BOOL,   0,  1,       false, "JCM_FFT_TILES",       nullptr},
+    {"fft_ywin",        &jcm_ctx::fft_ywin,        Option::BOOL,   0,  1,       false, "JCM_FFT_YWIN",        nullptr},
     {"fft_logits_rows", &jcm_ctx::fft_logits_rows, Option::BOOL,   0,  1,       false, "JCM_FFT_LOGITS_ROWS", nullptr},
     {"fft_reg",         &jcm_ctx::fft_reg,         Option::BOOL,   0,  1,       false, "JCM_FFT_REG",         nullptr},
     {"fft_cache_gb",    &jcm_ctx::fft_cache_gb,    Option::RANGE,  0,  1 << 20, false, "JCM_FFT_CACHE_GB",    nullptr},
```
